# xmindflow/TransCeption

Measured on AMD Instinct MI355X. Metric: images/sec fwd+bwd at 224x224 B=16 per GPU, higher is better.
Workload: dtype bf16; 1 GPU; TransCeption (MSTransception) 224x224 B=16/GPU fwd+bwd+SGD, synthetic Synapse npz slices via the device loader, name-seeded random-init weights; global_batch=16, image_size=224, parallelism=dp1, headline_mode=loader, headline_degraded=False, launch_mode=hipGraph replay

## Files before the change

### include/transception_hip.h

```cpp
#ifndef TRANSCEPTION_HIP_H
#define TRANSCEPTION_HIP_H

#ifdef __cplusplus
extern "C" {
#endif

enum { TC_OK = 0, TC_ERR_ARG = -1, TC_ERR_LAUNCH = -2, TC_ERR_UNSUPPORTED = -3 };
enum { TC_F32 = 0, TC_BF16 = 1, TC_F16 = 2 };
enum { TC_ACT_NONE = 0, TC_ACT_HSWISH = 1, TC_ACT_COORD = 2, TC_ACT_SIGMOID = 3, TC_ACT_GELU = 4,
       TC_ACT_SCALE = 5 ,
       TC_ACT_RELU = 6   };

int tc_abi_version(void);

typedef struct TcGemm {
    const void* A; const void* B; void* C;
    const void* bias;
    const void* R;
    int M, N, K;
    int lda, ldb, ldc, ldr;
    int transA, transB;
    int nb1, nb2;
    long long sA1, sA2, sB1, sB2, sC1, sC2, sR1, sR2;
    float alpha;
    int accumulate;
    int act;
    int splitk;
    int dtype;
    int c_f32;
    int atomic;
    float* rowsum;
    long long sBias1, sRow1;
    int bgap_every;
    long long bgap;
    void* ws;
    long long ws_bytes;
    int ffn_mode, ffn_nchunk, ffn_chunk_n, ffn_ldd;
    float ffn_eps;
    const float* ffn_part; float* ffn_stat; const void* ffn_gamma; const void* ffn_beta; const void* ffn_d; float* ffn_part2;
    long long ffn_sRow1, ffn_sPar1;
    void* ffn_aout;
    float* bn_part; const float* bn_shift;
} TcGemm;
enum { TC_FFN_NONE = 0, TC_FFN_LN_A = 1, TC_FFN_LN_B = 2, TC_FFN_EP = 3 };
int tc_gemm(const TcGemm* g, void* stream);
int tc_gemm_pair(const TcGemm* a, const TcGemm* b, void* stream);
int tc_gemm_multi(const TcGemm* g, int n, void* stream);

int tc_colsum(const void* x, int rows, int cols, int ldx, int nb, long long sb, float* out, int accumulate, int dtype,
              void* stream);

int tc_layernorm_fwd(const void* x, int ldx, const void* gamma, const void* beta, void* y, int ldy,
                     float* mean, float* rstd, int rows, int C, float eps, int act, int groups, long long pstride,
                     int dtype, void* stream);
int tc_layernorm_bwd(const void* dy, int lddy, const void* x, int ldx, const void* gamma, const void* beta,
                     const float* mean, const float* rstd, void* dx, int lddx, const void* dres, int ldres,
                     float* dgamma, float* dbeta, int rows, int C, int act, int groups, long long pstride,
                     float* scratch, long long scratch_floats, int dtype, void* stream);
long long tc_layernorm_bwd_scratch_floats(int rows, int C, int groups);
typedef struct {
    const float* part;
    float* dgamma; float* dbeta;
    long long pstride;
    int nblk, C, groups;
} TcLnFold;
int tc_layernorm_bwd_nblk(int rows, int C);
int tc_layernorm_bwd_defer(const void* dy, int lddy, const void* x, int ldx, const void* gamma, const void* beta,
                           const float* mean, const float* rstd, void* dx, int lddx, const void* dres, int ldres,
                           float* dgamma, float* dbeta, int rows, int C, int act, int groups, long long pstride,
                           float* part, long long part_floats, int dtype, void* stream);
int tc_layernorm_fold(const TcLnFold* sites, int n, void* stream);
int tc_layernorm_bwd_params(const void* dy, int lddy, const void* x, int ldx, const void* gamma, const void* beta,
                            const float* mean, const float* rstd, float* dgamma, float* dbeta, int rows, int C, int act,
                            int groups, long long pstride, int dtype, void* stream);

int tc_layernorm_ps_fwd(const void* x, int ldx, const void* gamma, const void* beta, void* y, int ldy, float* mean, float* rstd,
                        int B, int H, int W, int p, int C, float eps, int dtype, void* stream);
int tc_layernorm_ps_bwd(const void* dy, int lddy, const void* x, int ldx, const void* gamma, const void* beta, const float* mean,
                        const float* rstd, void* dx, int lddx, float* dgamma, float* dbeta, int B, int H, int W, int p, int C,
                        float* scratch, long long scratch_floats, int dtype, void* stream);

int tc_ln_cls_supported(int C, int ncls, int dtype);
long long tc_ln_cls_scratch_floats(int rows, int ncls);
int tc_ln_cls_fwd(const void* x, int ldx, const void* gamma, const void* beta, const void* Wc, const void* bc, void* logits, int ldl,
                  float* mean, float* rstd, int B, int H, int W, int p, int C, int ncls, float eps, int dtype, void* stream);
int tc_ln_cls_bwd(const void* dl, int lddl, const void* x, int ldx, const void* gamma, const void* beta, const void* Wc, const float* mean,
                  const float* rstd, void* dx, int lddx, float* dgamma, float* dbeta, float* dWc, float* dbc, float* scratch,
                  long long scratch_floats, int B, int H, int W, int p, int C, int ncls, int dtype, void* stream);

int tc_dwconv_fwd(const void* x, int ldx, const void* w, const void* bias, void* y, int ldy,
                  int B, int H, int W, int C, int k, int stride, int add_input, int groups, long long wstride, int dtype,
                  void* stream);
int tc_dwconv_bwd_input(const void* dy, int lddy, const void* w, void* dx, int lddx,
                        int B, int H, int W, int C, int k, int stride, int add_input, int accumulate, int groups,
                        long long wstride, int dtype, void* stream);
int tc_dwconv_bwd_weight(const void* dy, int lddy, const void* x, int ldx, float* dw, float* db,
                         int B, int H, int W, int C, int k, int stride, int groups, long long wstride, void* ws,
                         long long ws_bytes, int dtype, void* stream);
typedef struct {
    const float* part; float* dw; float* db;
    float* dgamma; float* dbeta;
    long long wstride;
    int C, k, groups;
    int ch, chunks, gx, nt;
} TcDwFold;
long long tc_dwconv_bwd_plan(int B, int H, int W, int C, int k, int groups, int dtype, TcDwFold* site);
int tc_dw_fold(const TcDwFold* sites, int n, void* stream);
int tc_dwconv_bwd(const void* dy, int lddy, const void* x, int ldx, const void* w, void* dx, int lddx, float* dw, float* db, int B, int H,
                  int W, int C, int k, int add_input, int accumulate, int groups, long long wstride, void* ws, long long ws_bytes,
                  int dtype, void* stream);

typedef struct TcDwSeg {
    const void* x; const void* w; const void* bias; void* y; const void* dy; float* dw; float* db;
    int C; int k; int ldx; int ldy; int lddy; int B; int H; int W;
    float* stat;
} TcDwSeg;
int tc_dwconv_multi(const TcDwSeg* segs, int nseg, int mode, int add_input, int accumulate, int groups, long long wstride,
                    void* ws, long long ws_bytes, int dtype, void* stream);
long long tc_dwconv_multi_plan(const TcDwSeg* segs, int nseg, int groups, int dtype, TcDwFold* sites, long long* offs);

int tc_ffn_chunk(int C, int dtype);
int tc_ffn_dw_fwd(const void* x, int ldx, const void* w, const void* bias, void* y, int ldy, float* stat, int B, int H, int W,
                  int C, int groups, long long wstride, int dtype, void* stream);
typedef struct TcFfnSeg {
    const void* gp; const void* d; const void* h; void* dh; const float* stat; const float* part2; const void* w; const void* gamma;
    float* dw; float* db; float* dgamma; float* dbeta;
    int C, ldg, ldd, ldh, lddh, B, H, W, nch2;
} TcFfnSeg;
int tc_ffn_mid_bwd(const TcFfnSeg* segs, int nseg, int groups, long long wstride, void* ws, long long ws_bytes, int dtype,
                   void* stream);
// ... 263 lines not shown
```

### transception_amd/_lib.py

```python
from __future__ import annotations

import ctypes as C
import os

HERE = os.path.dirname(os.path.abspath(__file__))
LIB_PATH = os.environ.get("TC_LIB_PATH") or os.path.join(HERE, "libtransception_hip.so")

TC_F32, TC_BF16, TC_F16 = 0, 1, 2
ACT_NONE, ACT_HSWISH, ACT_COORD, ACT_SIGMOID, ACT_GELU, ACT_SCALE, ACT_RELU = 0, 1, 2, 3, 4, 5, 6
ABI_VERSION = 15
ATTN_DKV_SPLITS = 8

vp, i32, i64, f32, f64 = C.c_void_p, C.c_int, C.c_longlong, C.c_float, C.c_double


class TcGemm(C.Structure):
    _fields_ = [("A", vp), ("B", vp), ("C", vp), ("bias", vp), ("R", vp),
                ("M", i32), ("N", i32), ("K", i32),
                ("lda", i32), ("ldb", i32), ("ldc", i32), ("ldr", i32),
                ("transA", i32), ("transB", i32), ("nb1", i32), ("nb2", i32),
                ("sA1", i64), ("sA2", i64), ("sB1", i64), ("sB2", i64),
                ("sC1", i64), ("sC2", i64), ("sR1", i64), ("sR2", i64),
                ("alpha", f32), ("accumulate", i32), ("act", i32), ("splitk", i32), ("dtype", i32), ("c_f32", i32), ("atomic", i32), ("rowsum", vp), ("sBias1", i64), ("sRow1", i64),
                ("bgap_every", i32), ("bgap", i64), ("ws", vp), ("ws_bytes", i64),
                ("ffn_mode", i32), ("ffn_nchunk", i32), ("ffn_chunk_n", i32), ("ffn_ldd", i32), ("ffn_eps", f32),
                ("ffn_part", vp), ("ffn_stat", vp), ("ffn_gamma", vp), ("ffn_beta", vp), ("ffn_d", vp), ("ffn_part2", vp),
                ("ffn_sRow1", i64), ("ffn_sPar1", i64), ("ffn_aout", vp),
                ("bn_part", vp), ("bn_shift", vp)]


FFN_NONE, FFN_LN_A, FFN_LN_B, FFN_EP = 0, 1, 2, 3


class TcDwSeg(C.Structure):
    _fields_ = [("x", vp), ("w", vp), ("bias", vp), ("y", vp), ("dy", vp), ("dw", vp), ("db", vp), ("C", i32), ("k", i32),
                ("ldx", i32), ("ldy", i32), ("lddy", i32), ("B", i32), ("H", i32), ("W", i32), ("stat", vp)]


class TcDwFold(C.Structure):
    _fields_ = [("part", vp), ("dw", vp), ("db", vp), ("dgamma", vp), ("dbeta", vp), ("wstride", i64), ("C", i32), ("k", i32), ("groups", i32),
                ("ch", i32), ("chunks", i32), ("gx", i32), ("nt", i32)]


class TcLnFold(C.Structure):
    _fields_ = [("part", vp), ("dgamma", vp), ("dbeta", vp), ("pstride", i64), ("nblk", i32), ("C", i32), ("groups", i32)]


class TcFfnSeg(C.Structure):
    _fields_ = [("gp", vp), ("d", vp), ("h", vp), ("dh", vp), ("stat", vp), ("part2", vp), ("w", vp), ("gamma", vp),
                ("dw", vp), ("db", vp), ("dgamma", vp), ("dbeta", vp),
                ("C", i32), ("ldg", i32), ("ldd", i32), ("ldh", i32), ("lddh", i32), ("B", i32), ("H", i32), ("W", i32), ("nch2", i32)]


class TcFfnFused(C.Structure):
    _fields_ = [("x", vp), ("w1", vp), ("b1", vp), ("wd", vp), ("bd", vp), ("gamma", vp), ("beta", vp), ("w2", vp), ("b2", vp),
                ("res", vp), ("out", vp), ("h", vp), ("d", vp), ("a", vp), ("stat", vp),
                ("sres", i64), ("sout", i64), ("wstride", i64),
                ("ldx", i32), ("ldr", i32), ("ldo", i32), ("C", i32), ("B", i32), ("H", i32), ("W", i32), ("groups", i32), ("eps", f32),
                ("tile_h", i32), ("tile_w", i32), ("pre_gamma", vp), ("pre_beta", vp), ("pre_eps", f32)]


class TcFfnBwd(C.Structure):
    _fields_ = [("x", vp), ("dy", vp), ("d", vp), ("stat", vp),
                ("w1", vp), ("b1", vp), ("wd", vp), ("gamma", vp), ("beta", vp), ("w2", vp),
                ("dx", vp), ("gd", vp), ("part", vp), ("part_floats", i64),
                ("dw1", vp), ("db1", vp), ("dwd", vp), ("dbd", vp), ("dgamma", vp), ("dbeta", vp), ("dw2", vp), ("db2", vp),
                ("sdy", i64), ("wstride", i64),
                ("ldx", i32), ("lddy", i32), ("lddx", i32), ("C", i32), ("B", i32), ("H", i32), ("W", i32), ("groups", i32), ("acc_dx", i32),
                ("eps", f32), ("tile_h", i32), ("tile_w", i32),
                ("pre_gamma", vp), ("pre_beta", vp), ("dpre_gamma", vp), ("dpre_beta", vp), ("pre_eps", f32)]


class TcEffAtt(C.Structure):
    _fields_ = [("t", vp), ("gamma", vp), ("beta", vp),
                ("wk", vp), ("bk", vp), ("wq", vp), ("bq", vp), ("wv", vp), ("bv", vp), ("wr", vp), ("br", vp),
                ("out", vp), ("ctx", vp), ("kstat", vp), ("part", vp), ("part_floats", i64),
                ("dout", vp), ("dt", vp), ("g1", vp),
                ("dgamma", vp), ("dbeta", vp), ("dwk", vp), ("dbk", vp), ("dwq", vp), ("dbq", vp), ("dwv", vp), ("dbv", vp), ("dwr", vp), ("dbr", vp),
                ("ldt", i32), ("ldo", i32), ("lddo", i32), ("lddt", i32), ("acc_dt", i32), ("C", i32), ("B", i32), ("N", i32),
                ("eps", f32)]


class TcEwSeg(C.Structure):
    _fields_ = [("kind", i32), ("flag", i32), ("a", vp), ("b", vp), ("sa", i64), ("sb", i64),
                ("lda", i32), ("ldb", i32), ("n0", i32), ("n1", i32), ("n2", i32), ("n3", i32), ("n4", i32), ("reserved", i32)]


EW_PATCHIFY, EW_DEINTERLEAVE, EW_COPY = 0, 1, 2


class TcSliceAug(C.Structure):
    _fields_ = [("m", C.c_double * 6), ("disp", C.c_float * 32), ("alpha", f32), ("center", f32), ("noise_sigma", f32),
                ("noise_seed", C.c_uint), ("flags", i32), ("reserved", i32)]


TC_AUG_WARP, TC_AUG_LINEAR, TC_AUG_BLUR, TC_AUG_PIECEWISE = 1, 2, 4, 8
TC_AUG_SKIP, TC_AUG_FROM_RAW = 1 << 20, 1 << 21
TC_METRIC_NO_SOURCE = 1 << 28
TC_METRIC_SELECT_WORK_BYTES = 16448

SIGNATURES = {
    "tc_abi_version": [],
    "tc_gemm": [C.POINTER(TcGemm), vp],
    "tc_ew_multi": [C.POINTER(TcEwSeg), i32, i32, vp],
    "tc_gemm_pair": [C.POINTER(TcGemm), C.POINTER(TcGemm), vp],
    "tc_gemm_multi": [C.POINTER(TcGemm), i32, vp],
    "tc_colsum": [vp, i32, i32, i32, i32, i64, vp, i32, i32, vp],
    "tc_layernorm_fwd": [vp, i32, vp, vp, vp, i32, vp, vp, i32, i32, f32, i32, i32, i64, i32, vp],
    "tc_layernorm_bwd": [vp, i32, vp, i32, vp, vp, vp, vp, vp, i32, vp, i32, vp, vp, i32, i32, i32, i32, i64, vp, i64, i32, vp],
    "tc_layernorm_bwd_scratch_floats": [i32, i32, i32],
    "tc_layernorm_bwd_nblk": [i32, i32],
    "tc_dwconv_bwd_plan": [i32, i32, i32, i32, i32, i32, i32, vp],
    "tc_dwconv_multi_plan": [vp, i32, i32, i32, vp, vp],
    "tc_ffn_mid_plan": [vp, i32, i32, i32, vp, vp],
    "tc_dw_fold": [vp, i32, vp],
    "tc_layernorm_bwd_defer": [vp, i32, vp, i32, vp, vp, vp, vp, vp, i32, vp, i32, vp, vp, i32, i32, i32, i32, i64, vp, i64, i32, vp],
    "tc_layernorm_fold": [vp, i32, vp],
    "tc_layernorm_ps_fwd": [vp, i32, vp, vp, vp, i32, vp, vp, i32, i32, i32, i32, i32, f32, i32, vp],
    "tc_layernorm_ps_bwd": [vp, i32, vp, i32, vp, vp, vp, vp, vp, i32, vp, vp, i32, i32, i32, i32, i32, vp, i64, i32, vp],
    "tc_ln_cls_supported": [i32, i32, i32],
    "tc_ln_cls_scratch_floats": [i32, i32],
    "tc_ln_cls_fwd": [vp, i32, vp, vp, vp, vp, vp, i32, vp, vp, i32, i32, i32, i32, i32, i32, f32, i32, vp],
    "tc_ln_cls_bwd": [vp, i32, vp, i32, vp, vp, vp, vp, vp, vp, i32, vp, vp, vp, vp, vp, i64, i32, i32, i32, i32, i32, i32, i32, vp],
    "tc_layernorm_bwd_params": [vp, i32, vp, i32, vp, vp, vp, vp, vp, vp, i32, i32, i32, i32, i64, i32, vp],
    "tc_dwconv_fwd": [vp, i32, vp, vp, vp, i32, i32, i32, i32, i32, i32, i32, i32, i32, i64, i32, vp],
    "tc_dwconv_bwd_input": [vp, i32, vp, vp, i32, i32, i32, i32, i32, i32, i32, i32, i32, i32, i64, i32, vp],
    "tc_dwconv_bwd_weight": [vp, i32, vp, i32, vp, vp, i32, i32, i32, i32, i32, i32, i32, i64, vp, i64, i32, vp],
    "tc_dwconv_bwd": [vp, i32, vp, i32, vp, vp, i32, vp, vp, i32, i32, i32, i32, i32, i32, i32, i32, i64, vp, i64, i32, vp],
    "tc_dwconv_multi": [C.POINTER(TcDwSeg), i32, i32, i32, i32, i32, i64, vp, i64, i32, vp],
    "tc_ffn_chunk": [i32, i32],
    "tc_ffn_dw_fwd": [vp, i32, vp, vp, vp, i32, vp, i32, i32, i32, i32, i32, i64, i32, vp],
    "tc_ffn_mid_bwd": [C.POINTER(TcFfnSeg), i32, i32, i64, vp, i64, i32, vp],
    "tc_ffn_fused_supported": [i32, i32],
    "tc_ffn_fused_fwd": [C.POINTER(TcFfnFused), i32, vp],
    "tc_ffn_fused_bwd_supported": [i32, i32],
    "tc_ffn_fused_bwd_scratch_floats": [i32, i32],
    "tc_ffn_fused_bwd": [C.POINTER(TcFfnBwd), i32, vp],
    "tc_effatt_supported": [i32, i32],
    "tc_effatt_scratch_floats": [i32, i32, i32],
    "tc_effatt_fwd": [C.POINTER(TcEffAtt), i32, vp],
    "tc_effatt_bwd": [C.POINTER(TcEffAtt), i32, vp],
    "tc_bn_scratch_floats": [i32, i32],
    "tc_bn_fwd": [vp, i32, vp, vp, vp, vp, vp, i32, vp, i32, vp, vp, vp, i32, i32, f32, f32, i32, i32, i32, i32, vp],
    "tc_bn_bwd": [vp, i32, vp, i32, vp, vp, vp, vp, vp, i32, vp, vp, vp, i32, i32, i32, i32, i32, vp],
    "tc_softmax_scratch_floats": [i32, i32, i32],
    "tc_softmax_fwd": [vp, vp, vp, i32, i64, i64, i32, i32, i32, i32, i32, i32, vp],
    "tc_softmax_bwd": [vp, vp, vp, vp, i32, i64, i64, i64, i32, i32, i32, i32, i32, i32, i32, i32, vp],
    "tc_attn_fwd": [vp, i32, i64, vp, i32, vp, i32, i64, vp, i32, i64, vp, i32, i32, i32, f32, i32, vp],
    "tc_attn_bwd": [vp, i32, i64, vp, i32, vp, i32, i64, vp, i32, i64, vp, i32, i64, vp, vp, vp, i32, i64, vp, i32,
                    vp, i32, i64, i32, i32, i32, i32, f32, i32, vp],
    "tc_attn_fwd_seg": [vp, i32, vp, i32, vp, i32, i64, vp, i32, vp, i32, i32, C.POINTER(i32), i32, f32, i32, i32, vp],
    "tc_attn_bwd_seg": [vp, i32, vp, i32, vp, i32, i64, vp, i32, vp, i32, vp, vp, vp, vp, i32, vp, i32, vp, i32, i64, i32, i32,
                        C.POINTER(i32), i32, f32, i32, i32, vp],
    "tc_fma3_fwd": [vp, i32, vp, i32, vp, i32, vp, i32, i32, i32, f32, i32, vp],
    "tc_fma3_bwd": [vp, i32, vp, i32, vp, i32, vp, i32, vp, i32, i32, vp, i32, i32, i32, f32, i32, vp],
    "tc_add": [vp, i32, vp, i32, vp, i32, i32, i32, i32, vp],
    "tc_sigmoid_bwd": [vp, vp, vp, i64, i32, vp],
    "tc_copy3d": [vp, i64, i32, vp, i64, i32, i32, i32, i32, i32, i32, vp],
    "tc_transpose": [vp, vp, i32, i32, i32, i32, vp],
    "tc_chan_pool_fwd": [vp, i32, vp, i32, i32, i32, i32, vp],
    "tc_chan_pool_bwd": [vp, vp, i32, i32, i32, i32, i32, i32, vp],
    "tc_chan_gate_fwd": [vp, i32, vp, vp, i32, i32, i32, i32, i32, vp],
    "tc_chan_gate_bwd": [vp, i32, vp, i32, vp, vp, i32, i32, vp, i32, i32, i32, i32, vp],
    "tc_relu_fwd": [vp, vp, i64, i32, vp],
    "tc_relu_bwd": [vp, vp, vp, i64, i32, vp],
    "tc_chan_pool2_fwd": [vp, i32, vp, vp, i32, i32, i32, i32, vp],
    "tc_chan_pool2_bwd": [vp, vp, vp, i32, i32, i32, i32, i32, i32, vp],
    "tc_pix_stats_fwd": [vp, i32, vp, vp, i32, i32, i32, vp],
    "tc_pix_stats_bwd": [vp, vp, vp, i32, i32, i32, i32, i32, vp],
    "tc_sa_conv_fwd": [vp, vp, vp, vp, i32, i32, i32, i32, i32, vp],
    "tc_sa_conv_bwd": [vp, vp, vp, vp, vp, vp, vp, i32, i32, i32, i32, i32, vp],
    "tc_pix_gate_fwd": [vp, i32, vp, vp, i32, i32, i32, i32, vp],
    "tc_pix_gate_bwd": [vp, i32, vp, i32, vp, vp, i32, i32, vp, i32, i32, i32, vp],
    "tc_cam_att_fwd": [vp, i32, vp, i32, i32, i32, i32, vp],
    "tc_cam_apply_fwd": [vp, i32, vp, vp, vp, i32, i32, i32, i32, i32, vp],
    "tc_cam_bwd": [vp, i32, vp, i32, vp, vp, vp, vp, vp, i32, i32, i32, i32, i32, i32, vp],
    "tc_gamma_res_fwd": [vp, i32, vp, i32, vp, vp, i32, i32, i32, i32, vp],
    "tc_gamma_res_bwd": [vp, i32, vp, i32, vp, vp, i32, vp, i32, i32, vp, i32, i32, i32, vp],
    "tc_gelu_fwd": [vp, vp, i64, i32, vp],
    "tc_gelu_bwd": [vp, vp, vp, i64, i32, vp],
    "tc_coord_pool_fwd": [vp, vp, i32, i32, i32, i32, i32, vp],
    "tc_coord_pool_bwd": [vp, vp, i32, i32, i32, i32, i32, i32, vp],
    "tc_coord_gate_fwd": [vp, vp, vp, i32, i32, i32, i32, i32, vp],
    "tc_coord_gate_bwd": [vp, vp, vp, vp, i32, vp, i32, i32, i32, i32, i32, vp],
    "tc_pixel_shuffle": [vp, vp, i32, i32, i32, i32, i32, i32, i32, vp],
    "tc_patchify": [vp, i64, i32, vp, i32, i32, i32, i32, i32, i32, i32, vp],
    "tc_sr_deinterleave": [vp, vp, i64, i32, i32, i32, i32, i32, i32, i32, vp],
    "tc_stem_im2col": [vp, vp, i32, i32, i32, i32, i32, i32, vp],
    "tc_window_rows": [vp, i32, vp, i32, i32, i32, i32, i32, i32, i32, i32, i32, i32, i32, vp],
    "tc_dropout": [vp, vp, i64, f32, vp, C.c_uint, i32, vp],
    "tc_im2col3s2": [vp, i32, i32, i32, vp, i32, i32, i32, i32, i32, i32, vp],
    "tc_col2im3s2": [vp, i32, vp, i32, i32, i32, i32, i32, i32, i32, vp],
    "tc_seg_loss_fwd": [vp, vp, vp, vp, i32, i32, i32, i32, vp],
    "tc_factor_att_stats_floats": [i32, i32, i32],
    "tc_factor_att_fwd": [vp, vp, vp, i32, vp, i32, vp, i32, vp, i32, i32, i32, i32, f32, i32, vp],
    "tc_factor_att_bwd": [vp, vp, vp, i32, vp, i32, vp, i32, vp, vp, vp, vp, i32, i32, i32, i32, vp, i32, i32, i32, i32, i32, f32, i32, vp],
    "tc_argmax_counts": [vp, vp, vp, vp, i32, i32, i32, i32, vp],
    "tc_metric_hist_bins": [i32, i32, i32],
    "tc_metric_surfaces": [vp, vp, vp, vp, vp, i32, i32, i32, i32, i32, vp],
    "tc_metric_edt": [vp, i32, vp, i32, i32, i32, i32, vp],
    "tc_metric_hist": [vp, vp, vp, vp, i32, vp, i64, i32, i32, i32, i32, vp],
    "tc_metric_select": [vp, i64, i32, vp, vp],
    "tc_metric_edt_f64": [vp, i32, vp, i32, i32, i32, i32, f64, f64, f64, vp],
    "tc_metric_select_f64": [vp, vp, vp, vp, i32, i32, i32, i32, i32, vp, vp, vp],
    "tc_seg_loss_bwd": [vp, vp, vp, vp, i32, i32, i32, f32, f32, f32, f32, vp, i32, vp],
    "tc_seg_loss_fwd_tok": [vp, i32, vp, vp, vp, i32, i32, i32, i32, vp],
    "tc_seg_loss_bwd_tok": [vp, vp, i32, vp, vp, vp, i32, i32, i32, i32, f32, f32, f32, f32, vp, i32, vp],
    "tc_seg_loss_value": [vp, i32, C.c_double, C.c_double, C.c_double, vp, vp],
    "tc_seg_loss_fwd_w": [vp, i32, vp, vp, i32, vp, vp, i32, i32, i32, i32, vp],
    "tc_seg_loss_value_w": [vp, vp, i32, C.c_double, C.c_double, vp, vp],
    "tc_seg_loss_bwd_w": [vp, vp, i32, vp, vp, i32, vp, vp, i32, i32, i32, i32, f32, f32, f32, vp, i32, vp],
    "tc_slice_augment": [vp, vp, vp, vp, vp, i32, i32, i32, vp],
    "tc_slice_augment_chain": [vp, vp, vp, i32, i32, vp, vp, vp, vp, i32, i32, i32, vp],
    "tc_spline_prefilter": [vp, vp, i32, i32, i32, vp],
    "tc_zoom_normalize": [vp, vp, vp, vp, vp, i32, i32, i32, i32, i32, f32, f32, vp],
    "tc_sgd_step": [vp, vp, vp, i64, f32, vp, f32, f32, f32, i32, vp],
    "tc_sgd_step_multi": [vp, vp, vp, vp, i32, i64, f32, vp, f32, f32, f32, i32, vp, f32, vp, i32, vp],
    "tc_sgd_step_multi_scaled": [vp, vp, vp, vp, i32, i64, f32, vp, f32, f32, f32, i32, vp, f32, vp, i32, vp, vp],
    "tc_loss_scale_update": [vp, vp, f32, f32, i32, f32, f32, vp],
    "tc_grad_sumsq": [vp, i64, vp, vp],
    "tc_fill_f32": [vp, i64, f32, vp],
    "tc_cast": [vp, vp, i64, i32, i32, vp],
    "tc_seg_marker": [i32, vp],
    "tc_im2col_dil": [vp, i32, vp, i32, i32, i32, i32, i32, i32, i32, i32, i32, i32, vp],
    "tc_col2im_dil": [vp, i32, vp, i32, i32, i32, i32, i32, i32, i32, i32, i32, i32, i32, vp],
    "tc_nearest_concat_fwd": [vp, i64, vp, i64, i32, vp, i32, i32, i32, i32, i32, i32, i32, i32, vp],
    "tc_nearest_concat_bwd": [vp, i32, vp, i64, vp, i64, i32, i32, i32, i32, i32, i32, i32, i32, i32, vp],
    "tc_linear_ln_supported": [i32, i32],
    "tc_linear_ln_fwd": [vp, i32, vp, vp, i64, vp, i32, vp, vp, i64, vp, i32, vp, i32, vp, vp, i32, i32, i32, f32, i32, vp],
    "tc_ripm_supported": [i32, i32],
    "tc_ripm_tiles": [i32, i32, i32],
    "tc_ripm_fwd": [vp, i32, i32, vp, i32, vp, vp, vp, vp, vp, vp, f32, f32, i32, vp, i32, vp, vp, vp, i32, vp, i32, vp, vp, i32, i32, i32, i32, i32, i32, vp],
    "tc_mhca_att_supported": [i32, i32, i32],
    "tc_dw_ln_supported": [i32, i32],
    "tc_dw_ln_fwd": [vp, i32, vp, vp, i64, vp, vp, i64, vp, i32, vp, i32, vp, vp, i32, i32, i32, i32, i32, f32, i32, vp],
    "tc_mhca_att_bwd_supported": [i32, i32, i32],
    "tc_mhca_att_bwd": [vp, i32, vp, i32, vp, i32, vp, vp, i32, i32, i32, i32, vp, vp, vp, vp, vp, vp, vp, vp, vp, i64, i32, i32, i32, i32, i32, f32, i32, vp],
    "tc_mhca_att_fwd": [vp, i32, vp, vp, vp, vp, vp, vp, vp, vp, i64, vp, i32, vp, i32, vp, i32, vp, i32, i32, i32, i32, i32, f32, i32, vp],
}
_RET = {"tc_ln_cls_scratch_floats": i64, "tc_ffn_fused_bwd_scratch_floats": i64, "tc_effatt_scratch_floats": i64, "tc_bn_scratch_floats": i64, "tc_softmax_scratch_floats": i64, "tc_layernorm_bwd_scratch_floats": i64, "tc_dwconv_bwd_plan": i64, "tc_dwconv_multi_plan": i64, "tc_ffn_mid_plan": i64, "tc_factor_att_stats_floats": i64, "tc_metric_hist_bins": i64}
_RAW = {"tc_abi_version", "tc_ln_cls_supported", "tc_ln_cls_scratch_floats", "tc_linear_ln_supported", "tc_ripm_supported", "tc_ripm_tiles", "tc_mhca_att_supported", "tc_dw_ln_supported", "tc_mhca_att_bwd_supported", "tc_effatt_supported", "tc_effatt_scratch_floats", "tc_ffn_chunk", "tc_ffn_fused_supported", "tc_ffn_fused_bwd_supported", "tc_ffn_fused_bwd_scratch_floats", "tc_bn_scratch_floats", "tc_softmax_scratch_floats", "tc_layernorm_bwd_scratch_floats", "tc_layernorm_bwd_nblk", "tc_dwconv_bwd_plan", "tc_dwconv_multi_plan", "tc_ffn_mid_plan", "tc_factor_att_stats_floats", "tc_metric_hist_bins"}


class TcError(RuntimeError):
    pass


class _Lib:
    calls = 0

    def __init__(self, path: str = LIB_PATH):
        if not os.path.exists(path):
            raise TcError(f"{path} is missing: build it with `python -m transception_amd.build` "
                          "(there is no CPU/PyTorch fallback for the TransCeption hot path)")
        self.path = path
        self.cdll = C.CDLL(path)
        for name, args in SIGNATURES.items():
            fn = getattr(self.cdll, name)
            fn.argtypes = args
            fn.restype = _RET.get(name, i32)
            setattr(self, name, fn if name in _RAW else self._checked(name, fn))
        v = self.cdll.tc_abi_version()
        if v != ABI_VERSION:
            raise TcError(f"ABI mismatch: library {v}, host {ABI_VERSION}")

    @staticmethod
    def _checked(name, fn):
        def call(*a):
            _Lib.calls += 1
            rc = fn(*a)
            if rc != 0:
                raise TcError(f"{name} failed with status {rc}")
        call.__name__ = name
        return call


_lib = None


def lib() -> _Lib:
    global _lib
    if _lib is None:
        _lib = _Lib()
    return _lib
```

### transception_amd/csrc/gemm.hip

```cpp
#include "tc_common.h"
#include <algorithm>
#include <type_traits>
#include <cstdlib>

typedef float f32x16 __attribute__((ext_vector_type(16)));
typedef __bf16 bf16x8 __attribute__((ext_vector_type(8)));
typedef _Float16 f16x8 __attribute__((ext_vector_type(8)));

template <typename H> struct HalfOps;
template <> struct HalfOps<bf16_t> {
    typedef bf16x8 v8;
    static __device__ __forceinline__ f32x16 mfma(v8 a, v8 b, f32x16 c) { return __builtin_amdgcn_mfma_f32_32x32x16_bf16(a, b, c, 0, 0, 0); }
};
template <> struct HalfOps<f16_t> {
    typedef f16x8 v8;
    static __device__ __forceinline__ f32x16 mfma(v8 a, v8 b, f32x16 c) { return __builtin_amdgcn_mfma_f32_32x32x16_f16(a, b, c, 0, 0, 0); }
};

namespace {

static inline unsigned fdiv_make(long long d, unsigned long long nmax) {
    return (d > 1 && nmax * (unsigned long long)d < (1ull << 32)) ? (unsigned)((1ull << 32) / (unsigned long long)d + 1) : 0u;
}
__device__ __forceinline__ int fdiv(int n, int d, unsigned m) { return d == 1 ? n : (m ? (int)__umulhi((unsigned)n, m) : n / d); }

struct GemmDev {
    const void* A; const void* B; void* C; const void* bias; const void* R;
    int M, N, K, lda, ldb, ldc, ldr;
    int nb2, splitk, kchunk;
    unsigned m_splitk, m_nb2, m_gx;
    long long sA1, sA2, sB1, sB2, sC1, sC2, sR1, sR2;
    float alpha; int accumulate, act;
    unsigned char vecA, vecB, vecC, atomic;
    short vec8C;
    short xcd;
    float* rowsum;
    long long sBias1, sRow1;
    float* ws_part; int* ws_cnt; short fix_group, fix_ngroups;
    int bgap_every; long long bgap;
    struct {
        int mode, nchunk, chunk_n, ldd, sRow1, sPar1;
        float eps;
        const float* part; float* stat; const void* gamma; const void* beta; const void* d; float* part2;
    } ffn;
    __device__ __host__ float* bn_part() const { return ffn.mode == 4 ? ffn.part2 : nullptr; }
    __device__ __host__ const float* bn_shift() const { return ffn.part; }
};
constexpr int GEMM_BN_STATS = 4;

template <typename H> __device__ __forceinline__ void bf8_unpack(const uint4& r, float* o) {
    unpack2<H>(r.x, o[0], o[1]); unpack2<H>(r.y, o[2], o[3]); unpack2<H>(r.z, o[4], o[5]); unpack2<H>(r.w, o[6], o[7]);
}
template <typename H> __device__ __forceinline__ uint4 bf8_pack(const float* o) {
    return make_uint4(pack2<H>(o[0], o[1]), pack2<H>(o[2], o[3]), pack2<H>(o[4], o[5]), pack2<H>(o[6], o[7]));
}
template <typename H> __device__ __forceinline__ uint4 ffn_ln_gelu8(const uint4& v, float mean, float rstd, const float* g, const float* b) {
    float x[8];
    bf8_unpack<H>(v, x);
#pragma unroll
    for (int e = 0; e < 8; e += 2) {
        const tc_f32x2 xv = {x[e], x[e + 1]}, gv = {g[e], g[e + 1]}, bv = {b[e], b[e + 1]};
        const tc_f32x2 u = gelu_poly2((xv - mean) * rstd * gv + bv);
        x[e] = u.x; x[e + 1] = u.y;
    }
    return bf8_pack<H>(x);
}
__device__ __forceinline__ float4 ffn_ln_gelu4(const float4& v, float mean, float rstd, const float4& g, const float4& b) {
    return make_float4(gelu_f((v.x - mean) * rstd * g.x + b.x), gelu_f((v.y - mean) * rstd * g.y + b.y),
                       gelu_f((v.z - mean) * rstd * g.z + b.z), gelu_f((v.w - mean) * rstd * g.w + b.w));
}
template <int BM>
__device__ __forceinline__ void ffn_finalize_stats(const GemmDev& p, int b1, int m0, bool write_out, float2* s_stat) {
    constexpr int LPR = 256 / BM;
    const int tid = threadIdx.x, r = tid / LPR, q = tid % LPR, row = m0 + r;
    const long long rbase = (long long)b1 * p.ffn.sRow1;
    const int nch = p.ffn.nchunk;
    const float cn = (float)p.ffn.chunk_n, inv_cn = 1.0f / cn, invC = 1.0f / (cn * (float)nch);
    const float2* pp = reinterpret_cast<const float2*>(p.ffn.part) + (rbase + (row < p.M ? row : 0)) * nch;
    float sm = 0.f, m2 = 0.f;
    constexpr int PMAX = 16;
    if (nch <= PMAX * LPR) {
        float2 t[PMAX];
#pragma unroll
        for (int e = 0; e < PMAX; ++e) t[e] = pp[min(q + e * LPR, nch - 1)];
#pragma unroll
        for (int e = 0; e < PMAX; ++e) if (q + e * LPR < nch) sm += t[e].x;
        sm = tc_group_sum<LPR>(sm);
        const float mean_ = sm * invC;
#pragma unroll
        for (int e = 0; e < PMAX; ++e) if (q + e * LPR < nch) { const float dm = t[e].x * inv_cn - mean_; m2 += t[e].y + cn * dm * dm; }
    } else {
        for (int k = q; k < nch; k += LPR) sm += pp[k].x;
        sm = tc_group_sum<LPR>(sm);
        const float mean_ = sm * invC;
        for (int k = q; k < nch; k += LPR) { const float2 t = pp[k]; const float dm = t.x * inv_cn - mean_; m2 += t.y + cn * dm * dm; }
    }
    const float mean = sm * invC;
    m2 = tc_group_sum<LPR>(m2);
    const float rstd = rsqrtf(m2 * invC + p.ffn.eps);
    if (q == 0) {
        s_stat[r] = make_float2(mean, rstd);
        if (write_out && row < p.M) reinterpret_cast<float2*>(p.ffn.stat)[rbase + row] = make_float2(mean, rstd);
    }
    __syncthreads();
}
template <typename T> __device__ __forceinline__ float ffn_ep1(float v, float d, float mean, float rstd, float g, float b, float& s1, float& s2) {
    const float xh = (d - mean) * rstd;
    const float gp = v * gelu_grad_fT<T>(xh * g + b);
    s1 += gp * g; s2 += gp * g * xh;
    return gp;
}

template <int TM, int TN>
__device__ __forceinline__ bool splitk_fixup(const GemmDev& p, f32x16 (&acc)[TM][TN], int tile, int ks, int& grp) {
    const int G = p.fix_group, tid = threadIdx.x;
    grp = ks / G;
    const int g0 = grp * G, gm = min(G, p.splitk - g0);
    if (gm == 1) return true;
    constexpr int NV = TM * TN * 16;
    float* part = p.ws_part + ((long long)tile * p.splitk + ks) * (NV * 256) + tid;
#pragma unroll
    for (int i = 0; i < TM; ++i)
#pragma unroll
        for (int j = 0; j < TN; ++j)
#pragma unroll
            for (int r = 0; r < 16; ++r)
                __hip_atomic_store(part + ((i * TN + j) * 16 + r) * 256, acc[i][j][r], __ATOMIC_RELAXED, __HIP_MEMORY_SCOPE_AGENT);
    __builtin_amdgcn_s_waitcnt(0);
    __builtin_amdgcn_fence(__ATOMIC_RELEASE, "workgroup");
    __syncthreads();
    __shared__ int s_last;
// ... 217 lines not shown
                    const int lr = part * 16 + r;
                    const float v = (m0 + lr < p.M) ? ldf<H>(stage + lr * LDS_ + cc) - sh : 0.f;
                    s1 += v; s2 += v * v;
                }
            }
            red[part * 64 + cc] = s1; red[256 + part * 64 + cc] = s2;
            __syncthreads();
            if (threadIdx.x < 64 && col < p.N) {
                const int T = (p.M + BM - 1) / BM, t = m0 / BM;
                bnp[p.N + (long long)t * p.N + col] = red[cc] + red[64 + cc] + red[128 + cc] + red[192 + cc];
                bnp[p.N + (long long)(T + t) * p.N + col] = red[256 + cc] + red[320 + cc] + red[384 + cc] + red[448 + cc];
                if (t == 0) bnp[col] = sh;
            }
        }
    }
}

template <typename H, int BM, int BN, int TM, int TN>
__device__ __forceinline__ void epilogue_rows_lds_ep(const GemmDev& p, f32x16 (&acc)[TM][TN], int b1, int m0, int n0, int wr, int wc, int lane,
                                                     bf16_t* stage_raw, const uint4 rd0, const uint4 rd1, int bx, int gx) {
    constexpr int LDS_ = BN + 8, WM = BM / 2, WN = BN / 2, CPR = BN / 8;
    H* stage = reinterpret_cast<H*>(stage_raw);
    H* dt = stage + BM * LDS_;
    float2* srow = reinterpret_cast<float2*>(dt + BM * LDS_);
    const long long rbase = (long long)b1 * p.ffn.sRow1;
    const H* gam = reinterpret_cast<const H*>(p.ffn.gamma) + (long long)b1 * p.ffn.sPar1;
    const H* bet = reinterpret_cast<const H*>(p.ffn.beta) + (long long)b1 * p.ffn.sPar1;
    const float2* stat = reinterpret_cast<const float2*>(p.ffn.stat) + rbase;
    const int h = lane >> 5;
    __syncthreads();
    {
        const int lr = threadIdx.x / CPR, lc = (threadIdx.x % CPR) * 8;
        *reinterpret_cast<uint4*>(dt + lr * LDS_ + lc) = rd0;
        *reinterpret_cast<uint4*>(dt + (lr + 256 / CPR) * LDS_ + lc) = rd1;
    }
    __syncthreads();
#pragma unroll
    for (int i = 0; i < TM; ++i) {
        const int lr = wr * WM + i * 32 + (lane & 31), row = m0 + lr;
        const float2 st = stat[row < p.M ? row : 0];
        float s1 = 0.f, s2 = 0.f;
#pragma unroll
        for (int j = 0; j < TN; ++j)
#pragma unroll
            for (int g = 0; g < 4; ++g) {
                const int lc = wc * WN + j * 32 + 8 * g + 4 * h, col = n0 + lc;
                float v[4];
#pragma unroll
                for (int e = 0; e < 4; ++e) v[e] = p.alpha * acc[i][j][4 * g + e];
                if (row < p.M && col < p.N) {
                    const float4 d4 = ld4<H>(dt + lr * LDS_ + lc), g4 = ld4<H>(gam + col), b4 = ld4<H>(bet + col);
                    {
                        const tc_f32x2 va = {v[0], v[1]}, vb = {v[2], v[3]};
                        const tc_f32x2 ga = {g4.x, g4.y}, gb = {g4.z, g4.w};
                        const tc_f32x2 xa = (tc_f32x2{d4.x, d4.y} - st.x) * st.y, xb = (tc_f32x2{d4.z, d4.w} - st.x) * st.y;
                        const tc_f32x2 pa = va * gelu_grad_f2_fast(xa * ga + tc_f32x2{b4.x, b4.y});
                        const tc_f32x2 pb = vb * gelu_grad_f2_fast(xb * gb + tc_f32x2{b4.z, b4.w});
                        const tc_f32x2 qa = pa * ga, qb = pb * gb, ra = qa * xa, rb = qb * xb;
                        s1 += (qa.x + qa.y) + (qb.x + qb.y);
                        s2 += (ra.x + ra.y) + (rb.x + rb.y);
                        v[0] = pa.x; v[1] = pa.y; v[2] = pb.x; v[3] = pb.y;
                    }
                }
                st4<H>(stage + lr * LDS_ + lc, make_float4(v[0], v[1], v[2], v[3]));
            }
        s1 += __shfl_xor(s1, 32, 64); s2 += __shfl_xor(s2, 32, 64);
        if (h == 0) srow[wc * BM + lr] = make_float2(s1, s2);
    }
    __syncthreads();
    H* C = reinterpret_cast<H*>(p.C) + b1 * p.sC1;
#pragma unroll
    for (int it = 0; it < BM * CPR / 256; ++it) {
        const int idx = threadIdx.x + it * 256, lr = idx / CPR, lc = (idx - lr * CPR) * 8;
        const int row = m0 + lr, col = n0 + lc;
        if (row < p.M && col < p.N)
            *reinterpret_cast<uint4*>(C + (long long)row * p.ldc + col) = *reinterpret_cast<const uint4*>(stage + lr * LDS_ + lc);
    }
    if (threadIdx.x < BM && m0 + threadIdx.x < p.M) {
        const float2 a = srow[threadIdx.x], b = srow[BM + threadIdx.x];
        reinterpret_cast<float2*>(p.ffn.part2)[(rbase + m0 + threadIdx.x) * gx + bx] = make_float2(a.x + b.x, a.y + b.y);
    }
}

__device__ __forceinline__ float4 load_strip(const float* base, int ld, int x, int k, int X, int K, bool trans, bool vec) {
    float4 v = make_float4(0.f, 0.f, 0.f, 0.f);
    if (!trans) {
        if (x < X) {
            const float* p = base + (long long)x * ld + k;
            if (vec && k + 3 < K) v = *reinterpret_cast<const float4*>(p);
            else {
                if (k + 0 < K) v.x = p[0];
                if (k + 1 < K) v.y = p[1];
                if (k + 2 < K) v.z = p[2];
                if (k + 3 < K) v.w = p[3];
            }
        }
    } else {
        if (k < K) {
            const float* p = base + (long long)k * ld + x;
            if (vec && x + 3 < X) v = *reinterpret_cast<const float4*>(p);
            else {
                if (x + 0 < X) v.x = p[0];
                if (x + 1 < X) v.y = p[1];
                if (x + 2 < X) v.z = p[2];
                if (x + 3 < X) v.w = p[3];
            }
        }
    }
    return v;
}

template <typename TC, int BM, int BN, bool TA, bool TB, int FFN = 0>
__global__ __launch_bounds__(256) void gemm_kernel(GemmDev p) {
    constexpr int BK = 16, LDT = BK + 1;
    constexpr int WM = BM / 2, WN = BN / 2, TM = WM / 32, TN = WN / 32;
    constexpr int SA = BM * BK / 4 / 256, SB = BN * BK / 4 / 256;
    static_assert(SA >= 1 && SB >= 1, "tile too small");
    static_assert(FFN == 0 || (BM == 64 && BN == 64), "the MixFFN hooks run on 64x64 tiles");
    static_assert(FFN != TC_FFN_LN_A || !TA, "LN_A transforms rows of a row-major A");
    static_assert(FFN != TC_FFN_LN_B || !TB, "LN_B transforms rows of a [K,N] B");
    __shared__ float As[BM * LDT];
    __shared__ float Bs[BN * LDT];
    __shared__ float2 s_ffn[FFN ? 2 * 64 : 1];

    const int tid = threadIdx.x, lane = tid & 63, wave = tid >> 6;
    const int wr = wave >> 1, wc = wave & 1;
    int z = blockIdx.z;
    const int ks = z % p.splitk; z /= p.splitk;
    const int b2 = z % p.nb2, b1 = z / p.nb2;
    const int m0 = blockIdx.y * BM, n0 = blockIdx.x * BN;
    const int kbeg = ks * p.kchunk;
    const int kend = min(p.K, kbeg + p.kchunk);

    const float* A = reinterpret_cast<const float*>(p.A) + b1 * p.sA1 + b2 * p.sA2;
    const float* B = reinterpret_cast<const float*>(p.B) + b1 * p.sB1 + b2 * p.sB2;
    const float* gam = FFN ? reinterpret_cast<const float*>(p.ffn.gamma) + (long long)b1 * p.ffn.sPar1 : nullptr;
    const float* bet = FFN ? reinterpret_cast<const float*>(p.ffn.beta) + (long long)b1 * p.ffn.sPar1 : nullptr;
    const float2* fstat = FFN ? reinterpret_cast<const float2*>(p.ffn.stat) + (long long)b1 * p.ffn.sRow1 : nullptr;

    f32x16 acc[TM][TN];
#pragma unroll
    for (int i = 0; i < TM; ++i)
#pragma unroll
        for (int j = 0; j < TN; ++j)
#pragma unroll
            for (int r = 0; r < 16; ++r) acc[i][j][r] = 0.f;

    float a_mean = 0.f, a_rstd = 0.f;
    float4 hg = make_float4(0.f, 0.f, 0.f, 0.f), hb = hg;
    float2 hst = make_float2(0.f, 0.f);
    if constexpr (FFN == TC_FFN_LN_A) {
        ffn_finalize_stats<BM>(p, b1, m0, blockIdx.x == 0 && ks == 0, s_ffn);
        const float2 st = s_ffn[tid / (BK / 4)];
        a_mean = st.x; a_rstd = st.y;
    }
    if constexpr (FFN == TC_FFN_LN_B) {
        const int col = n0 + (tid % (BN / 4)) * 4;
        if (col + 3 < p.N) { hg = *reinterpret_cast<const float4*>(gam + col); hb = *reinterpret_cast<const float4*>(bet + col); }
    }

    float4 ra[SA], rb[SB];
    auto fetch = [&](int k0) __attribute__((always_inline)) {
#pragma unroll
        for (int i = 0; i < SA; ++i) {
            const int f = tid + i * 256;
            if (!TA) { const int row = f / (BK / 4), kq = f % (BK / 4);
// ... 60 lines not shown
        if (k0 + BK < kend) fetch(k0 + BK);
        if (do_rowsum) {
#pragma unroll
            for (int kk = 0; kk < BK; ++kk) rsum += As[tid * LDT + kk];
        }
        const float* ap = &As[(wr * WM + (lane & 31)) * LDT + (lane >> 5)];
        const float* bp = &Bs[(wc * WN + (lane & 31)) * LDT + (lane >> 5)];
#pragma unroll
        for (int kk = 0; kk < BK; kk += 2) {
            float a[TM], b[TN];
#pragma unroll
            for (int i = 0; i < TM; ++i) a[i] = ap[i * 32 * LDT + kk];
#pragma unroll
            for (int j = 0; j < TN; ++j) b[j] = bp[j * 32 * LDT + kk];
#pragma unroll
            for (int i = 0; i < TM; ++i)
#pragma unroll
                for (int j = 0; j < TN; ++j)
                    acc[i][j] = __builtin_amdgcn_mfma_f32_32x32x2f32(a[i], b[j], acc[i][j], 0, 0, 0);
        }
        __syncthreads();
    }
    if (do_rowsum && m0 + tid < p.M) atomicAdd(p.rowsum + b1 * p.sRow1 + m0 + tid, rsum);
    bool first = (ks == 0), atomic = p.atomic;
    if (p.fix_group) {
        int grp;
        if (!splitk_fixup<TM, TN>(p, acc, (int)(((blockIdx.z / p.splitk) * gridDim.y + blockIdx.y) * gridDim.x + blockIdx.x), ks, grp)) return;
        first = (grp == 0); atomic = p.fix_ngroups > 1;
    }
    if constexpr (FFN == TC_FFN_EP)
        epilogue_cols<float, TC, TM, TN, true>(p, acc, b1, b2, first, atomic, m0 + wr * WM, n0 + wc * WN, lane, s_ffn, wr * WM, wc, m0,
                                               (int)blockIdx.x, (int)gridDim.x);
    else
        epilogue_cols<float, TC, TM, TN>(p, acc, b1, b2, first, atomic, m0 + wr * WM, n0 + wc * WN, lane);
}

__device__ __forceinline__ bool strip_whole(int x, int k, int X, int K, bool trans) {
    return trans ? (k < K && x + 7 < X) : (x < X && k + 7 < K);
}
__device__ __forceinline__ uint4 strip_raw(const bf16_t* base, const bf16_t* safe, int ld, int x, int k, int X, int K, bool trans) {
    const long long off = trans ? (long long)k * ld + x : (long long)x * ld + k;
    return *reinterpret_cast<const uint4*>(strip_whole(x, k, X, K, trans) ? base + off : safe);
}
__device__ __forceinline__ uint4 strip_tail(const bf16_t* base, int ld, int x, int k, int X, int K, bool trans) {
    union { uint4 v; bf16_t e[8]; } u;
    u.v = make_uint4(0u, 0u, 0u, 0u);
    const bf16_t* p = base + (trans ? (long long)k * ld + x : (long long)x * ld + k);
#pragma unroll
    for (int i = 0; i < 8; ++i) if (trans ? (x + i < X) : (k + i < K)) u.e[i] = p[i];
    return u.v;
}
__device__ __forceinline__ uint4 load_strip8(const bf16_t* base, int ld, int x, int k, int X, int K, bool trans, bool vec) {
    const bool in = trans ? (k < K) : (x < X);
    if (!in) return make_uint4(0u, 0u, 0u, 0u);
    if (vec && strip_whole(x, k, X, K, trans))
        return *reinterpret_cast<const uint4*>(base + (trans ? (long long)k * ld + x : (long long)x * ld + k));
    return strip_tail(base, ld, x, k, X, K, trans);
}

__device__ __forceinline__ int gemm_krow(int k) { return (k & ~15) | ((k & 3) << 2) | ((k >> 2) & 3); }
typedef short s16x4_t __attribute__((ext_vector_type(4)));
typedef short s16x8_t __attribute__((ext_vector_type(8)));
template <typename V8> __device__ __forceinline__ V8 ld_frag_tr(const bf16_t* lo, const bf16_t* hi) {
    const s16x4_t a = __builtin_amdgcn_ds_read_tr16_b64_v4i16((s16x4_t __attribute__((address_space(3)))*)(lo));
    const s16x4_t b = __builtin_amdgcn_ds_read_tr16_b64_v4i16((s16x4_t __attribute__((address_space(3)))*)(hi));
    return __builtin_bit_cast(V8, (s16x8_t)__builtin_shufflevector(a, b, 0, 1, 2, 3, 4, 5, 6, 7));
}

#ifdef TC_GEMM_TIMING
__device__ unsigned long long g_gemm_dbg[1024 * 8];
__device__ unsigned int g_gemm_dbg_n;
#define GSTAMP(k) do { if (gs_ >= 0) { const long long t_ = __builtin_readcyclecounter(); g_gemm_dbg[gs_ * 8 + 1 + (k)] = (unsigned long long)(t_ - gt_); gt_ = t_; } } while (0)
#define GSTAMP_INIT() int gs_ = -1; long long gt_ = 0; \
    if (threadIdx.x == 0 && (blockIdx.x + 7 * blockIdx.y + 13 * blockIdx.z) % 61 == 0) { gs_ = (int)(atomicAdd(&g_gemm_dbg_n, 1u) & 1023u); \
        g_gemm_dbg[gs_ * 8] = (TA ? 4 : 0) + (TB ? 2 : 0) + (sizeof(TC) == 4 ? 1 : 0) + 8 * FFN + 1000ull * (unsigned long long)((kend_for_stamp)); gt_ = __builtin_readcyclecounter(); }
#else
#define GSTAMP(k)
#define GSTAMP_INIT()
#endif
template <typename H, typename TC, int BM, int BN, bool TA, bool TB, bool DB, int FFN = 0>
__device__ __forceinline__ void gemm_bf16_body(const GemmDev& p, const int bx, const int by, const int bz, const int gx, const int gy,
                                               bf16_t (*As)[BM * (64 + 8)], bf16_t (*Bs)[BN * (64 + 8)]) {
    constexpr int BK = 64, LDT = BK + 8;
    static_assert(FFN == 0 || (BM == 64 && BN == 64 && DB), "the MixFFN hooks run on 64x64 tiles with the double-buffered LDS");
    static_assert(FFN != TC_FFN_LN_A || !TA, "LN_A transforms rows of a row-major A");
    static_assert(FFN != TC_FFN_LN_B || !TB, "LN_B transforms rows of a [K,N] B");
    static_assert(FFN != TC_FFN_EP || sizeof(TC) == 2, "EP writes a bf16 C");
    constexpr bool SWAP = sizeof(TC) == 2;
    constexpr int WM = BM / 2, WN = BN / 2, TM = WM / 32, TN = WN / 32;
    constexpr int SA = BM * BK / 8 / 256, SB = BN * BK / 8 / 256;
    static_assert(SA >= 1 && SB >= 1, "tile too small");

    const int tid = threadIdx.x, lane = tid & 63, wave = tid >> 6;
    const int wr = wave >> 1, wc = wave & 1;
    int z = bz;
    const int zq = fdiv(z, p.splitk, p.m_splitk);
    const int ks = z - zq * p.splitk; z = zq;
    const int b1 = fdiv(z, p.nb2, p.m_nb2), b2 = z - b1 * p.nb2;
    const int m0 = by * BM, n0 = bx * BN;
    const int kbeg = ks * p.kchunk;
    const int kend = min(p.K, kbeg + p.kchunk);
    const int kend_for_stamp = kend - kbeg; (void)kend_for_stamp;
    GSTAMP_INIT();

    const bf16_t* A = reinterpret_cast<const bf16_t*>(p.A) + b1 * p.sA1 + b2 * p.sA2;
    const bf16_t* B = reinterpret_cast<const bf16_t*>(p.B) + b1 * p.sB1 + b2 * p.sB2;

    f32x16 acc[TM][TN];
#pragma unroll
    for (int i = 0; i < TM; ++i)
#pragma unroll
        for (int j = 0; j < TN; ++j)
#pragma unroll
            for (int r = 0; r < 16; ++r) acc[i][j][r] = 0.f;

    auto a_xy = [&](int i, int k0, int& x, int& k) __attribute__((always_inline)) {
        const int f = tid + i * 256;
        if (!TA) { x = m0 + f / (BK / 8); k = k0 + (f % (BK / 8)) * 8; }
        else { k = k0 + f / (BM / 8); x = m0 + (f % (BM / 8)) * 8; }
    };
    auto b_xy = [&](int i, int k0, int& x, int& k) __attribute__((always_inline)) {
        const int f = tid + i * 256;
        if (TB) { x = n0 + f / (BK / 8); k = k0 + (f % (BK / 8)) * 8; }
        else { k = k0 + f / (BN / 8); x = n0 + (f % (BN / 8)) * 8; }
    };
    auto b_base = [&](int k0) __attribute__((always_inline)) { return (!TB && p.bgap_every) ? B + (long long)(k0 / p.bgap_every) * p.bgap : B; };
    const bf16_t* gam = FFN ? reinterpret_cast<const bf16_t*>(p.ffn.gamma) + (long long)b1 * p.ffn.sPar1 : nullptr;
    const bf16_t* bet = FFN ? reinterpret_cast<const bf16_t*>(p.ffn.beta) + (long long)b1 * p.ffn.sPar1 : nullptr;
    const float2* fstat = FFN ? reinterpret_cast<const float2*>(p.ffn.stat) + (long long)b1 * p.ffn.sRow1 : nullptr;
    __shared__ float2 s_ffn[FFN == TC_FFN_LN_A ? BM : 1];
    float a_mean[SA], a_rstd[SA], fg[8], fb[8];
    bf16_t* aout = (FFN == TC_FFN_LN_A && p.ffn.d && bx == 0) ? reinterpret_cast<bf16_t*>(const_cast<void*>(p.ffn.d)) + (long long)b1 * p.ffn.sRow1 * p.ffn.ldd
                                                               : nullptr;
    uint4 rd0 = make_uint4(0u, 0u, 0u, 0u), rd1 = rd0;
    if constexpr (FFN == TC_FFN_LN_A) {
        ffn_finalize_stats<BM>(p, b1, m0, bx == 0 && ks == 0, s_ffn);
#pragma unroll
        for (int i = 0; i < SA; ++i) { const float2 st = s_ffn[(tid + i * 256) / (BK / 8)]; a_mean[i] = st.x; a_rstd[i] = st.y; }
    }
    if constexpr (FFN == TC_FFN_LN_B) {
        const int col = n0 + (tid % (BN / 8)) * 8;
        const int cc = col + 7 < p.N ? col : 0;
        bf8_unpack<H>(*reinterpret_cast<const uint4*>(gam + cc), fg);
        bf8_unpack<H>(*reinterpret_cast<const uint4*>(bet + cc), fb);
    }
    if constexpr (FFN == TC_FFN_EP) {
        const bf16_t* dmap = reinterpret_cast<const bf16_t*>(p.ffn.d) + (long long)b1 * p.ffn.sRow1 * p.ffn.ldd;
        static_assert(BM * BN / 8 / 256 == 2 || FFN != TC_FFN_EP, "two pieces per thread");
        const int lr = tid / (BN / 8), lc = (tid % (BN / 8)) * 8;
        const bool in0 = m0 + lr < p.M && n0 + lc < p.N, in1 = m0 + lr + 256 / (BN / 8) < p.M && n0 + lc < p.N;
        rd0 = *reinterpret_cast<const uint4*>(in0 ? dmap + (long long)(m0 + lr) * p.ffn.ldd + n0 + lc : dmap);
        rd1 = *reinterpret_cast<const uint4*>(in1 ? dmap + (long long)(m0 + lr + 256 / (BN / 8)) * p.ffn.ldd + n0 + lc : dmap);
    }
    auto fetch = [&](auto FT, uint4 (&ra)[SA], uint4 (&rb)[SB], uint4 (&rh)[2], int k0) __attribute__((always_inline)) {
        constexpr bool FAST = decltype(FT)::value;
        int x, k;
#pragma unroll
        for (int i = 0; i < SA; ++i) {
            a_xy(i, k0, x, k);
            if constexpr (FAST) ra[i] = strip_raw(A, A, p.lda, x, k, p.M, kend, TA);
            else ra[i] = load_strip8(A, p.lda, x, k, p.M, kend, TA, p.vecA);
        }
        const bf16_t* Bk = b_base(k0);
#pragma unroll
        for (int i = 0; i < SB; ++i) {
            b_xy(i, k0, x, k);
            if constexpr (FAST) rb[i] = strip_raw(Bk, B, p.ldb, x, k, p.N, kend, !TB);
// ... 44 lines not shown
            else if constexpr (FFN == TC_FFN_LN_B) { if (!strip_whole(x, k, p.N, kend, !TB)) v = make_uint4(0u, 0u, 0u, 0u); }
            if (TB) { const int row = f / (BK / 8), kq = f % (BK / 8); *reinterpret_cast<uint4*>(&bs[row * LDT + kq * 8]) = v; }
            else { const int kl = f / (BN / 8), nq = f % (BN / 8); *reinterpret_cast<uint4*>(&bs[gemm_krow(kl) * PB + nq * 8]) = v; }
        }
    };
    float rsum = 0.f;
    const bool do_rowsum = p.rowsum && bx == 0 && tid < BM;
    auto compute = [&](const bf16_t* as, const bf16_t* bs) __attribute__((always_inline)) {
        if (do_rowsum) {
#pragma unroll
            for (int kk = 0; kk < BK; ++kk) rsum += ldf<H>(reinterpret_cast<const H*>(TA ? as + kk * PA + tid : as + tid * LDT + kk));
        }
        const int h = lane >> 5, gi = lane & 15, gq = (lane >> 4) & 1;
        const bf16_t* ap = TA ? &as[(2 * h + 4 * (gi >> 2)) * PA + wr * WM + 16 * gq + 4 * (gi & 3)] : &as[(wr * WM + (lane & 31)) * LDT + 8 * h];
        const bf16_t* bp = !TB ? &bs[(2 * h + 4 * (gi >> 2)) * PB + wc * WN + 16 * gq + 4 * (gi & 3)] : &bs[(wc * WN + (lane & 31)) * LDT + 8 * h];
#pragma unroll
        for (int kk = 0; kk < BK; kk += 16) {
            typedef typename HalfOps<H>::v8 V8;
            V8 a[TM], b[TN];
#pragma unroll
            for (int i = 0; i < TM; ++i) {
                if constexpr (TA) a[i] = ld_frag_tr<V8>(ap + kk * PA + i * 32, ap + (kk + 1) * PA + i * 32);
                else a[i] = *reinterpret_cast<const V8*>(ap + i * 32 * LDT + kk);
            }
#pragma unroll
            for (int j = 0; j < TN; ++j) {
                if constexpr (!TB) b[j] = ld_frag_tr<V8>(bp + kk * PB + j * 32, bp + (kk + 1) * PB + j * 32);
                else b[j] = *reinterpret_cast<const V8*>(bp + j * 32 * LDT + kk);
            }
#pragma unroll
            for (int i = 0; i < TM; ++i)
#pragma unroll
                for (int j = 0; j < TN; ++j)
                    acc[i][j] = SWAP ? HalfOps<H>::mfma(b[j], a[i], acc[i][j])
                                     : HalfOps<H>::mfma(a[i], b[j], acc[i][j]);
        }
    };

    auto kloop = [&](auto FT) __attribute__((always_inline)) {
    constexpr bool FAST = decltype(FT)::value;
    uint4 ra0[SA], rb0[SB], ra1[SA], rb1[SB], rh0[2], rh1[2];
    if (!DB) {
        if (kbeg < kend) fetch(FT, ra0, rb0, rh0, kbeg);
        for (int k0 = kbeg; k0 < kend; k0 += BK) {
            stage(FT, ra0, rb0, rh0, k0, As[0], Bs[0]);
            __syncthreads();
            if (k0 + BK < kend) fetch(FT, ra0, rb0, rh0, k0 + BK);
            compute(As[0], Bs[0]);
            __syncthreads();
        }
    } else if (kbeg < kend) {
        fetch(FT, ra0, rb0, rh0, kbeg);
        if (FAST || kbeg + BK < kend) fetch(FT, ra1, rb1, rh1, kbeg + BK);
        stage(FT, ra0, rb0, rh0, kbeg, As[0], Bs[0]);
        __syncthreads();
        if (FAST || kbeg + 2 * BK < kend) fetch(FT, ra0, rb0, rh0, kbeg + 2 * BK);
        for (int k0 = kbeg;; k0 += 2 * BK) {
            const bool has1 = k0 + BK < kend;
            if (has1) stage(FT, ra1, rb1, rh1, k0 + BK, As[DB ? 1 : 0], Bs[DB ? 1 : 0]);
            compute(As[0], Bs[0]);
            if (!has1) break;
            __syncthreads();
            if (FAST || k0 + 3 * BK < kend) fetch(FT, ra1, rb1, rh1, k0 + 3 * BK);
            const bool has2 = k0 + 2 * BK < kend;
            if (has2) stage(FT, ra0, rb0, rh0, k0 + 2 * BK, As[0], Bs[0]);
            compute(As[DB ? 1 : 0], Bs[DB ? 1 : 0]);
            if (!has2) break;
            __syncthreads();
            if (FAST || k0 + 4 * BK < kend) fetch(FT, ra0, rb0, rh0, k0 + 4 * BK);
        }
    }
    };
    const bool fast = p.vecA && p.vecB && ((kend - kbeg) % 8 == 0 || (TA && !TB)) && (!TA || p.M % 8 == 0) && (TB || p.N % 8 == 0);
    GSTAMP(0);
    if (fast) kloop(std::true_type{}); else kloop(std::false_type{});
    GSTAMP(1);
    if (do_rowsum && m0 + tid < p.M) atomicAdd(p.rowsum + b1 * p.sRow1 + m0 + tid, rsum);
    bool first = (ks == 0), atomic = p.atomic;
    if (p.fix_group) {
        int grp;
        if (!splitk_fixup<TM, TN>(p, acc, (zq * gy + by) * gx + bx, ks, grp)) return;
        first = (grp == 0); atomic = p.fix_ngroups > 1;
    }
    if constexpr (FFN == TC_FFN_EP) {
        static_assert(FFN != TC_FFN_EP || 2 * BM * (BN + 8) + 2 * BM * 4 <= 2 * (BM + BN) * (64 + 8), "C stage + d tile + row sums must fit");
        epilogue_rows_lds_ep<H, BM, BN, TM, TN>(p, acc, b1, m0, n0, wr, wc, lane, &As[0][0], rd0, rd1, bx, gx);
    } else if constexpr (SWAP) {
        if (p.vec8C && !p.accumulate && !atomic && first) {
            static_assert((BM * (BN + 8)) <= (DB ? 2 : 1) * (BM + BN) * (64 + 8), "staging tile must fit the operand buffers");
            epilogue_rows_lds<H, BM, BN, TM, TN>(p, acc, b1, b2, m0, n0, wr, wc, lane, &As[0][0]);
        } else {
            epilogue_rows<H, TC, TM, TN>(p, acc, b1, b2, first, atomic, m0 + wr * WM, n0 + wc * WN, lane);
        }
    } else {
        epilogue_cols<H, TC, TM, TN>(p, acc, b1, b2, first, atomic, m0 + wr * WM, n0 + wc * WN, lane);
    }
    GSTAMP(2);
}

__device__ __forceinline__ void tc_xcd_tile(int& bx, int& by, const int gx, const int gy, const unsigned mgx) {
    const int T = gx * gy, L = bx + gx * by;
    const int xcd = L & 7, slot = L >> 3, q = T >> 3, r = T & 7;
    const int t = xcd * q + min(xcd, r) + slot;
    by = fdiv(t, gx, mgx);
    bx = t - by * gx;
}

#ifndef GEMM_OCC64
#define GEMM_OCC64 5
#endif
template <typename H, typename TC, int BM, int BN, bool TA, bool TB, bool DB, int FFN = 0>
__global__ __launch_bounds__(256, (BM == 64 && BN == 64) ? GEMM_OCC64 : 2) void gemm_bf16_kernel(GemmDev p) {
    __shared__ __attribute__((aligned(16))) bf16_t smem[(DB ? 2 : 1) * (BM + BN) * (64 + 8)];
    int tbx = blockIdx.x, tby = blockIdx.y;
    if (p.xcd & 1) tc_xcd_tile(tbx, tby, gridDim.x, gridDim.y, p.m_gx);
    gemm_bf16_body<H, TC, BM, BN, TA, TB, DB, FFN>(p, tbx, tby, blockIdx.z, gridDim.x, gridDim.y,
                                                reinterpret_cast<bf16_t(*)[BM * (64 + 8)]>(smem),
                                                reinterpret_cast<bf16_t(*)[BN * (64 + 8)]>(smem + (DB ? 2 : 1) * BM * (64 + 8)));
}

struct GemmPairDev { GemmDev a, b; int nA, gxA, gyA, gxB, gyB; unsigned mgxA, mgyA, mgxB, mgyB; };
template <typename H>
__global__ __launch_bounds__(256, 2) void gemm_pair_kernel(GemmPairDev q) {
    __shared__ __attribute__((aligned(16))) bf16_t smem[2 * (64 + 64) * (64 + 8)];
    bf16_t(*As)[64 * (64 + 8)] = reinterpret_cast<bf16_t(*)[64 * (64 + 8)]>(smem);
    bf16_t(*Bs)[64 * (64 + 8)] = reinterpret_cast<bf16_t(*)[64 * (64 + 8)]>(smem + 2 * 64 * (64 + 8));
    const int nB = (int)gridDim.x - q.nA;
    int lin = (int)blockIdx.x < nB ? (int)blockIdx.x + q.nA : (int)blockIdx.x - nB;
    if (lin < q.nA) {
        const int l1 = fdiv(lin, q.gxA, q.mgxA);
        int bx = lin - l1 * q.gxA;
        const int bz = fdiv(l1, q.gyA, q.mgyA);
        int by = l1 - bz * q.gyA;
        if (q.a.xcd & 1) tc_xcd_tile(bx, by, q.gxA, q.gyA, q.mgxA);
        if (q.a.ffn.mode == TC_FFN_EP) gemm_bf16_body<H, H, 64, 64, false, false, true, TC_FFN_EP>(q.a, bx, by, bz, q.gxA, q.gyA, As, Bs);
        else gemm_bf16_body<H, H, 64, 64, false, false, true>(q.a, bx, by, bz, q.gxA, q.gyA, As, Bs);
    } else {
        lin -= q.nA;
        if (q.b.xcd & 2) {
            const int xcd = lin & 7, slot = lin >> 3, qq = nB >> 3, r = nB & 7;
            lin = xcd * qq + min(xcd, r) + slot;
        }
        const int l1 = fdiv(lin, q.gxB, q.mgxB), bx = lin - l1 * q.gxB, bz = fdiv(l1, q.gyB, q.mgyB), by = l1 - bz * q.gyB;
        if (q.b.ffn.mode == TC_FFN_LN_B) gemm_bf16_body<H, float, 64, 64, true, false, true, TC_FFN_LN_B>(q.b, bx, by, bz, q.gxB, q.gyB, As, Bs);
        else gemm_bf16_body<H, float, 64, 64, true, false, true>(q.b, bx, by, bz, q.gxB, q.gyB, As, Bs);
    }
}

constexpr int GEMM_MULTI_MAX = 12;
static_assert(sizeof(GemmDev) * GEMM_MULTI_MAX + 20 * GEMM_MULTI_MAX + 8 <= 4096, "kernel argument block");
struct GemmMultiDev { GemmDev p[GEMM_MULTI_MAX]; int blk0[GEMM_MULTI_MAX], gx[GEMM_MULTI_MAX], gy[GEMM_MULTI_MAX], kind[GEMM_MULTI_MAX]; unsigned mgy[GEMM_MULTI_MAX]; int n; };
template <typename H>
__global__ __launch_bounds__(256, 4) void gemm_multi_kernel(GemmMultiDev q) {
    __shared__ __attribute__((aligned(16))) bf16_t smem[2 * (64 + 64) * (64 + 8)];
    bf16_t(*As)[64 * (64 + 8)] = reinterpret_cast<bf16_t(*)[64 * (64 + 8)]>(smem);
    bf16_t(*Bs)[64 * (64 + 8)] = reinterpret_cast<bf16_t(*)[64 * (64 + 8)]>(smem + 2 * 64 * (64 + 8));
    int lin = blockIdx.x, i = 0;
    for (int j = 1; j < q.n; ++j) if (lin >= q.blk0[j]) i = j;
    lin -= q.blk0[i];
    if (q.p[i].xcd & 2) {
        const int ni = (i + 1 < q.n ? q.blk0[i + 1] : (int)gridDim.x) - q.blk0[i];
        const int xcd = lin & 7, slot = lin >> 3, qq = ni >> 3, r = ni & 7;
        lin = xcd * qq + min(xcd, r) + slot;
    }
    const int gx = q.gx[i], gy = q.gy[i];
    const unsigned mgx = q.p[i].m_gx;
    const int l1 = fdiv(lin, gx, mgx), bz = fdiv(l1, gy, q.mgy[i]);
    int bx = lin - l1 * gx, by = l1 - bz * gy;
    if ((q.p[i].xcd & 1) && q.kind[i] != 2 && q.kind[i] != 5) tc_xcd_tile(bx, by, gx, gy, mgx);
    const GemmDev p = q.p[i];
    if (q.kind[i] == 0) gemm_bf16_body<H, H, 64, 64, false, true, true>(p, bx, by, bz, gx, gy, As, Bs);
    else if (q.kind[i] == 1) gemm_bf16_body<H, H, 64, 64, false, false, true>(p, bx, by, bz, gx, gy, As, Bs);
    else if (q.kind[i] == 2) gemm_bf16_body<H, float, 64, 64, true, false, true>(p, bx, by, bz, gx, gy, As, Bs);
    else if (q.kind[i] == 3) gemm_bf16_body<H, H, 64, 64, false, true, true, TC_FFN_LN_A>(p, bx, by, bz, gx, gy, As, Bs);
    else if (q.kind[i] == 4) gemm_bf16_body<H, H, 64, 64, false, false, true, TC_FFN_EP>(p, bx, by, bz, gx, gy, As, Bs);
    else gemm_bf16_body<H, float, 64, 64, true, false, true, TC_FFN_LN_B>(p, bx, by, bz, gx, gy, As, Bs);
}

template <typename T, typename TC, int BM, int BN, bool TA, bool TB>
void launch_one(const GemmDev& d, dim3 grid, hipStream_t s) {
    if constexpr (sizeof(T) == 4) hipLaunchKernelGGL((gemm_kernel<TC, BM, BN, TA, TB>), grid, dim3(256), 0, s, d);
    else if (d.kchunk > 128) hipLaunchKernelGGL((gemm_bf16_kernel<T, TC, BM, BN, TA, TB, true>), grid, dim3(256), 0, s, d);
    else hipLaunchKernelGGL((gemm_bf16_kernel<T, TC, BM, BN, TA, TB, false>), grid, dim3(256), 0, s, d);
}

template <typename T>
int launch_ffn(const GemmDev& d, dim3 grid, hipStream_t s) {
    if constexpr (sizeof(T) == 4) {
        if (d.ffn.mode == TC_FFN_LN_A) hipLaunchKernelGGL((gemm_kernel<float, 64, 64, false, true, TC_FFN_LN_A>), grid, dim3(256), 0, s, d);
        else if (d.ffn.mode == TC_FFN_LN_B) hipLaunchKernelGGL((gemm_kernel<float, 64, 64, true, false, TC_FFN_LN_B>), grid, dim3(256), 0, s, d);
        else hipLaunchKernelGGL((gemm_kernel<float, 64, 64, false, false, TC_FFN_EP>), grid, dim3(256), 0, s, d);
    } else {
        if (d.ffn.mode == TC_FFN_LN_A) hipLaunchKernelGGL((gemm_bf16_kernel<T, T, 64, 64, false, true, true, TC_FFN_LN_A>), grid, dim3(256), 0, s, d);
        else if (d.ffn.mode == TC_FFN_LN_B) hipLaunchKernelGGL((gemm_bf16_kernel<T, float, 64, 64, true, false, true, TC_FFN_LN_B>), grid, dim3(256), 0, s, d);
        else hipLaunchKernelGGL((gemm_bf16_kernel<T, T, 64, 64, false, false, true, TC_FFN_EP>), grid, dim3(256), 0, s, d);
    }
    return tc_launch_status();
}

template <typename T, typename TC, int BM, int BN>
int launch(const GemmDev& d, int transA, int transB, dim3 grid, hipStream_t s) {
    if (!transA && transB) launch_one<T, TC, BM, BN, false, true>(d, grid, s);
    else if (!transA && !transB) launch_one<T, TC, BM, BN, false, false>(d, grid, s);
    else if (transA && !transB) launch_one<T, TC, BM, BN, true, false>(d, grid, s);
    else launch_one<T, TC, BM, BN, true, true>(d, grid, s);
    return tc_launch_status();
}

template <typename T>
bool gemm_plan(const TcGemm* g, GemmDev& d, dim3& grid, bool& use128_out, bool force64 = false) {
    d.A = g->A; d.B = g->B; d.C = g->C; d.bias = g->bias; d.R = g->R;
    d.M = g->M; d.N = g->N; d.K = g->K; d.lda = g->lda; d.ldb = g->ldb; d.ldc = g->ldc; d.ldr = g->ldr;
    d.nb2 = g->nb2; d.splitk = g->splitk;
    d.sA1 = g->sA1; d.sA2 = g->sA2; d.sB1 = g->sB1; d.sB2 = g->sB2;
    d.sC1 = g->sC1; d.sC2 = g->sC2; d.sR1 = g->sR1; d.sR2 = g->sR2;
    d.alpha = g->alpha; d.accumulate = g->accumulate; d.act = g->act;
    d.rowsum = g->rowsum;
    d.sBias1 = g->sBias1; d.sRow1 = g->sRow1;
    d.bgap_every = g->bgap_every; d.bgap = g->bgap;
    d.ffn.mode = g->ffn_mode; d.ffn.nchunk = g->ffn_nchunk; d.ffn.chunk_n = g->ffn_chunk_n; d.ffn.ldd = g->ffn_ldd;
    d.ffn.sRow1 = (int)g->ffn_sRow1; d.ffn.sPar1 = (int)g->ffn_sPar1; d.ffn.eps = g->ffn_eps;
    d.ffn.part = g->ffn_part; d.ffn.stat = g->ffn_stat; d.ffn.gamma = g->ffn_gamma; d.ffn.beta = g->ffn_beta;
    d.ffn.d = g->ffn_mode == TC_FFN_LN_A ? g->ffn_aout : g->ffn_d;
    d.ffn.part2 = g->ffn_part2;
    if (g->bn_part && !g->ffn_mode) { d.ffn.mode = GEMM_BN_STATS; d.ffn.part2 = g->bn_part; d.ffn.part = g->bn_shift; }
    if (g->ffn_mode || g->bn_part) force64 = true;
    constexpr int VEC = 16 / (int)sizeof(T);
    auto aligned = [&](const void* ptr, int ld, long long s1, long long s2) {
        return ((uintptr_t)ptr % 16 == 0) && (ld % VEC == 0) && (s1 % VEC == 0) && (s2 % VEC == 0);
    };
    d.vecA = aligned(g->A, g->lda, g->sA1, g->sA2);
    d.vecB = aligned(g->B, g->ldb, g->sB1, g->sB2);
    {
        const int csz = g->c_f32 ? 4 : (int)sizeof(T);
        const bool cok = ((uintptr_t)g->C % (4 * csz) == 0) && (g->ldc % 4 == 0) && (g->sC1 % 4 == 0) && (g->sC2 % 4 == 0);
        const bool rok = !g->R || (((uintptr_t)g->R % (4 * sizeof(T)) == 0) && (g->ldr % 4 == 0) && (g->sR1 % 4 == 0) && (g->sR2 % 4 == 0));
        d.vecC = cok && rok;
        d.vec8C = !g->c_f32 && sizeof(T) == 2 && cok && rok && ((uintptr_t)g->C % 16 == 0) && (g->ldc % 8 == 0) && (g->sC1 % 8 == 0) &&
                  (g->sC2 % 8 == 0) && (g->N % 8 == 0);
    }
    const int nb = g->nb1 * g->nb2;
    const long long big = (long long)((g->M + 127) / 128) * ((g->N + 127) / 128) * nb;
    constexpr long long thr128 = 100000;
    const bool use128 = !force64 && big >= thr128 && g->M >= 96 && g->N >= 96;
    const int BM = use128 ? 128 : 64, BN = use128 ? 128 : 64;
    constexpr int BK = sizeof(T) == 4 ? 16 : 64;
    constexpr int CNT_BYTES = 16384, PART_BYTES = 64 * 64 * 4, FIX_GROUP = 16;
    const long long tiles64 = (long long)((g->M + 63) / 64) * ((g->N + 63) / 64) * nb;
    const long long slots = (g->ws && g->ws_bytes > CNT_BYTES && (uintptr_t)g->ws % 16 == 0) ? (g->ws_bytes - CNT_BYTES) / PART_BYTES : 0;
    int want = g->splitk;
    bool fix = false;
    if (!use128 && slots > 0) {
#ifndef GEMM_AS_TILES
#define GEMM_AS_TILES 384
#define GEMM_AS_TARGET 512
#define GEMM_AS_KPER 256
#endif
        if (want == 1 && !g->atomic && g->ffn_mode != TC_FFN_EP && !g->bn_part && g->K >= 2 * GEMM_AS_KPER && tiles64 <= GEMM_AS_TILES) {
            long long sk = GEMM_AS_TARGET / tiles64;
            if (sk > g->K / GEMM_AS_KPER) sk = g->K / GEMM_AS_KPER;
            if (sk > FIX_GROUP) sk = FIX_GROUP;
            if (sk >= 2 && tiles64 * sk <= slots) { want = (int)sk; fix = true; }
        } else if (want > 128) {
            fix = tiles64 * want <= slots && tiles64 * ((want + FIX_GROUP - 1) / FIX_GROUP) <= CNT_BYTES / 4;
        }
    }
    int kchunk = (g->K + want - 1) / want;
    kchunk = (kchunk + BK - 1) / BK * BK;
    d.kchunk = kchunk;
    d.splitk = (g->K + kchunk - 1) / kchunk;
    if (d.splitk < 1) d.splitk = 1;
    d.fix_group = 0; d.fix_ngroups = 1; d.ws_part = nullptr; d.ws_cnt = nullptr;
    if (fix && d.splitk > 1) {
        d.fix_group = FIX_GROUP;
        d.fix_ngroups = (d.splitk + FIX_GROUP - 1) / FIX_GROUP;
        d.ws_cnt = reinterpret_cast<int*>(g->ws);
        d.ws_part = reinterpret_cast<float*>(reinterpret_cast<char*>(g->ws) + CNT_BYTES);
    }
    d.atomic = ((d.splitk > 1 && !d.fix_group) || g->atomic) ? 1 : 0;
    grid = dim3((g->N + BN - 1) / BN, (g->M + BM - 1) / BM, nb * d.splitk);
    d.m_splitk = fdiv_make(d.splitk, 65536); d.m_nb2 = fdiv_make(d.nb2, 65536);
    d.m_gx = fdiv_make(grid.x, (unsigned long long)grid.x * grid.y * grid.z);
    d.xcd = (grid.x > 1 && (long long)grid.x * grid.y >= 64) ? 1 : 0;
    use128_out = use128;
    if (g->bn_part) {
        if (sizeof(T) != 2 || g->c_f32 || g->accumulate || g->atomic || d.splitk != 1 || nb != 1 || !d.vec8C || g->ffn_mode || g->act != TC_ACT_NONE)
            return false;
    }
    if (g->ffn_mode) {
        if (!d.vecA || !d.vecB || (g->ffn_mode != TC_FFN_LN_B && g->K % VEC) || g->N % VEC || g->nb2 != 1 || (uintptr_t)g->ffn_gamma % 16 || (uintptr_t)g->ffn_beta % 16 ||
            g->ffn_sPar1 % VEC)
            return false;
        if (g->ffn_mode == TC_FFN_LN_A && (g->transA || !g->transB || g->c_f32 || g->K != g->ffn_nchunk * g->ffn_chunk_n ||
                                           (g->ffn_aout && ((uintptr_t)g->ffn_aout % 16 || g->ffn_ldd % VEC))))
            return false;
        if (g->ffn_mode == TC_FFN_LN_B && (!g->transA || g->transB || !(g->c_f32 || sizeof(T) == 4))) return false;
        if (g->ffn_mode == TC_FFN_EP && (g->transA || g->transB || g->c_f32 || g->accumulate || g->atomic || d.splitk != 1 || g->bias || g->R ||
                                         g->act != TC_ACT_NONE || (sizeof(T) == 2 && !d.vec8C) || (uintptr_t)g->ffn_d % 16 || g->ffn_ldd % VEC))
            return false;
    }
    return grid.y <= 65535 && grid.z <= 65535;
}

template <typename T>
int gemm_typed(const TcGemm* g, hipStream_t s) {
    GemmDev d;
    dim3 grid;
    bool use128;
    if (!gemm_plan<T>(g, d, grid, use128)) return TC_ERR_ARG;
    if (g->ffn_mode) return launch_ffn<T>(d, grid, s);
    if (g->c_f32)
        return use128 ? launch<T, float, 128, 128>(d, g->transA, g->transB, grid, s)
                      : launch<T, float, 64, 64>(d, g->transA, g->transB, grid, s);
    return use128 ? launch<T, T, 128, 128>(d, g->transA, g->transB, grid, s)
                  : launch<T, T, 64, 64>(d, g->transA, g->transB, grid, s);
}


}

static bool gemm_args_ok(const TcGemm* g) {
    if (!g || !g->A || !g->B || !g->C || g->M <= 0 || g->N <= 0 || g->K <= 0 || g->nb1 < 1 || g->nb2 < 1 || g->splitk < 1) return false;
    if ((g->splitk > 1 || g->atomic) && (!g->accumulate || (g->dtype != TC_F32 && !g->c_f32) || g->act != TC_ACT_NONE)) return false;
    if (g->act != TC_ACT_NONE && g->act != TC_ACT_SIGMOID && g->act != TC_ACT_SCALE) return false;
    if (g->act == TC_ACT_SCALE && g->ffn_mode != TC_FFN_NONE) return false;
    if (g->bgap_every < 0 || (g->bgap_every > 0 && (g->transB || g->bgap_every % 64 || (g->bgap % 8)))) return false;
    if (g->ffn_mode < TC_FFN_NONE || g->ffn_mode > TC_FFN_EP) return false;
    if (g->ffn_mode != TC_FFN_NONE) {
        if (!g->ffn_gamma || !g->ffn_beta || !g->ffn_stat || g->bgap_every) return false;
        if (g->ffn_mode == TC_FFN_LN_A && (!g->ffn_part || g->ffn_nchunk < 1 || g->ffn_chunk_n < 1)) return false;
        if (g->ffn_mode == TC_FFN_EP && (!g->ffn_d || !g->ffn_part2)) return false;
        if (g->ffn_sRow1 < 0 || g->ffn_sRow1 > 0x7fffffffLL || g->ffn_sPar1 < 0 || g->ffn_sPar1 > 0x7fffffffLL) return false;
    }
    return true;
}

#ifdef TC_GEMM_TIMING
extern "C" int tc_gemm_dbg_read(unsigned long long* dst, int reset) {
    int rc = (int)hipMemcpyFromSymbol(dst, HIP_SYMBOL(g_gemm_dbg), sizeof(unsigned long long) * 1024 * 8);
    if (reset) {
        static unsigned long long z[1024 * 8];
        unsigned int zn = 0;
        rc |= (int)hipMemcpyToSymbol(HIP_SYMBOL(g_gemm_dbg), z, sizeof(z));
        rc |= (int)hipMemcpyToSymbol(HIP_SYMBOL(g_gemm_dbg_n), &zn, sizeof(zn));
    }
    return rc;
}
#endif
extern "C" int tc_gemm(const TcGemm* g, void* stream) {
    if (!gemm_args_ok(g)) return TC_ERR_ARG;
    hipStream_t s = (hipStream_t)stream;
    TC_DISPATCH_DTYPE(g->dtype, return gemm_typed<T>(g, s));
    return TC_ERR_ARG;
}

extern "C" int tc_gemm_pair(const TcGemm* a, const TcGemm* b, void* stream) {
    if (!gemm_args_ok(a) || !gemm_args_ok(b) || a->bn_part || b->bn_part) return TC_ERR_ARG;
    hipStream_t s = (hipStream_t)stream;
    if ((a->dtype == TC_BF16 || a->dtype == TC_F16) && b->dtype == a->dtype && !a->transA && !a->transB && !a->c_f32 && b->transA && !b->transB && b->c_f32 &&
        (a->ffn_mode == TC_FFN_NONE || a->ffn_mode == TC_FFN_EP) && (b->ffn_mode == TC_FFN_NONE || b->ffn_mode == TC_FFN_LN_B)) {
        GemmPairDev q;
        dim3 ga, gb;
        bool bigA, bigB;
        if (!gemm_plan<bf16_t>(a, q.a, ga, bigA) || !gemm_plan<bf16_t>(b, q.b, gb, bigB)) return TC_ERR_ARG;
        const long long nA = (long long)ga.x * ga.y * ga.z, nB = (long long)gb.x * gb.y * gb.z;
        if (!bigA && !bigB && nA + nB < 0x7fffffffLL) {
            q.nA = (int)nA; q.gxA = ga.x; q.gyA = ga.y; q.gxB = gb.x; q.gyB = gb.y;
            q.mgxA = fdiv_make(ga.x, nA + nB); q.mgyA = fdiv_make(ga.y, nA + nB); q.mgxB = fdiv_make(gb.x, nA + nB); q.mgyB = fdiv_make(gb.y, nA + nB);
            if (gb.x * gb.y > 1) q.b.xcd |= 2;
            if (a->dtype == TC_BF16) hipLaunchKernelGGL(gemm_pair_kernel<bf16_t>, dim3((unsigned)(nA + nB)), dim3(256), 0, s, q);
            else hipLaunchKernelGGL(gemm_pair_kernel<f16_t>, dim3((unsigned)(nA + nB)), dim3(256), 0, s, q);
            return tc_launch_status();
        }
    }
    const int rc = tc_gemm(a, stream);
    return rc != TC_OK ? rc : tc_gemm(b, stream);
}

extern "C" int tc_gemm_multi(const TcGemm* g, int n, void* stream) {
    if (!g || n < 1) return TC_ERR_ARG;
    for (int i = 0; i < n; ++i) if (!gemm_args_ok(g + i) || g[i].bn_part) return TC_ERR_ARG;
    hipStream_t s = (hipStream_t)stream;
    bool ok = n <= GEMM_MULTI_MAX;
    GemmMultiDev q;
    GemmDev plan[GEMM_MULTI_MAX];
    dim3 grids[GEMM_MULTI_MAX];
    int kinds[GEMM_MULTI_MAX], order[GEMM_MULTI_MAX];
    for (int i = 0; ok && i < n; ++i) {
        const TcGemm& t = g[i];
        int kind = -1;
        const bool h16 = (t.dtype == TC_BF16 || t.dtype == TC_F16) && t.dtype == g[0].dtype;
        if (h16 && !t.transA && t.transB && !t.c_f32) kind = t.ffn_mode == TC_FFN_LN_A ? 3 : (t.ffn_mode ? -1 : 0);
        else if (h16 && !t.transA && !t.transB && !t.c_f32) kind = t.ffn_mode == TC_FFN_EP ? 4 : (t.ffn_mode ? -1 : 1);
        else if (h16 && t.transA && !t.transB && t.c_f32) kind = t.ffn_mode == TC_FFN_LN_B ? 5 : (t.ffn_mode ? -1 : 2);
        bool big;
        if (kind < 0 || !gemm_plan<bf16_t>(&t, plan[i], grids[i], big, true)) { ok = false; break; }
        kinds[i] = kind; order[i] = i;
    }
    long long blk = 0;
    if (ok) {
        std::stable_sort(order, order + n, [&](int a, int b) { return plan[a].kchunk > plan[b].kchunk; });
        for (int j = 0; j < n; ++j) {
            const int i = order[j];
            q.p[j] = plan[i]; q.kind[j] = kinds[i]; q.gx[j] = grids[i].x; q.gy[j] = grids[i].y; q.blk0[j] = (int)blk;
            q.mgy[j] = fdiv_make(grids[i].y, (unsigned long long)grids[i].x * grids[i].y * grids[i].z);
            if ((kinds[i] == 2 || kinds[i] == 5) && grids[i].x * grids[i].y > 1) q.p[j].xcd |= 2;
            blk += (long long)grids[i].x * grids[i].y * grids[i].z;
            if (blk > 0x7fffffffLL) ok = false;
        }
    }
    if (ok) {
        q.n = n;
        if (g[0].dtype == TC_BF16) hipLaunchKernelGGL(gemm_multi_kernel<bf16_t>, dim3((unsigned)blk), dim3(256), 0, s, q);
        else hipLaunchKernelGGL(gemm_multi_kernel<f16_t>, dim3((unsigned)blk), dim3(256), 0, s, q);
        return tc_launch_status();
    }
    for (int i = 0; i < n; ++i) {
        const int rc = tc_gemm(g + i, stream);
        if (rc != TC_OK) return rc;
    }
    return TC_OK;
}
```

### transception_amd/csrc/norm.hip

```cpp
#include "tc_common.h"
#include <cstdlib>

namespace {

constexpr int LN_MAXC = 2048;
#ifndef LN_FOLD
#define LN_FOLD 8
#endif
constexpr int LN_BWD_MAX_BLOCKS = 4096, LN_BWD_ROWS_PER_GROUP = 4;
constexpr int LN_BWD_WG_MIN = 1024;
inline int ln_bwd_blocks(bool deferred) {
    return deferred ? LN_BWD_MAX_BLOCKS : 1024;
}

struct LnMap { int p, H, W; };
__device__ __forceinline__ long long ln_row_off(int row, const LnMap& m, int ld, int C) {
    if (m.p == 0) return (long long)row * ld;
    const int Wp = m.W * m.p, Hp = m.H * m.p;
    const int ow = row % Wp, t = row / Wp, oh = t % Hp, b = t / Hp;
    return ((long long)(b * m.H + oh / m.p) * m.W + ow / m.p) * ld + ((oh % m.p) * m.p + ow % m.p) * C;
}

template <int GS> __device__ __forceinline__ float group_sum(float v) { return tc_group_sum<GS>(v); }

template <typename T, int GS, int NV, int RPT>
__global__ __launch_bounds__(256) void ln_fwd_kernel(const T* __restrict__ x, int ldx, const T* __restrict__ gamma,
                                                     const T* __restrict__ beta, T* __restrict__ y, int ldy,
                                                     float* __restrict__ mean, float* __restrict__ rstd, int rows,
                                                     int C, float eps, int act, long long pstride, LnMap map) {
    constexpr int RPB = 256 / GS;
    const int gl = threadIdx.x % GS, gi = threadIdx.x / GS;
    const int sst = (rstd == mean + 1) ? 2 : 1;
    {
        const long long g = blockIdx.y;
        x += g * rows * ldx; y += g * rows * ldy; mean += g * rows * sst; rstd += g * rows * sst; gamma += g * pstride; beta += g * pstride;
    }
    const int nv = C >> 2;
    const float invC = 1.0f / (float)C;
    float4 g[NV], b[NV];
#pragma unroll
    for (int i = 0; i < NV; ++i) {
        const int q = gl + i * GS;
        if (q < nv) { g[i] = ld4<T>(gamma + q * 4); b[i] = ld4<T>(beta + q * 4); }
    }
    for (int row0 = (blockIdx.x * RPB + gi) * RPT; row0 < rows; row0 += gridDim.x * RPB * RPT) {
        float4 v[RPT][NV];
        float mu[RPT], rs[RPT];
#pragma unroll
        for (int r = 0; r < RPT; ++r) {
            const int row = min(row0 + r, rows - 1);
            const T* xr = x + ln_row_off(row, map, ldx, C);
#pragma unroll
            for (int i = 0; i < NV; ++i) {
                const int q = gl + i * GS;
                v[r][i] = q < nv ? ld4<T>(xr + q * 4) : make_float4(0.f, 0.f, 0.f, 0.f);
            }
        }
#pragma unroll
        for (int r = 0; r < RPT; ++r) {
            float s = 0.f;
#pragma unroll
            for (int i = 0; i < NV; ++i) s += v[r][i].x + v[r][i].y + v[r][i].z + v[r][i].w;
            mu[r] = group_sum<GS>(s) * invC;
            float s2 = 0.f;
#pragma unroll
            for (int i = 0; i < NV; ++i) {
                const int q = gl + i * GS;
                if (q < nv) {
                    const float a = v[r][i].x - mu[r], bb = v[r][i].y - mu[r], c = v[r][i].z - mu[r], d = v[r][i].w - mu[r];
                    s2 += a * a + bb * bb + c * c + d * d;
                }
            }
            rs[r] = rsqrtf(group_sum<GS>(s2) * invC + eps);
        }
#pragma unroll
        for (int r = 0; r < RPT; ++r) {
            const int row = row0 + r;
            if (row >= rows) break;
            if (gl == 0) { mean[(long long)row * sst] = mu[r]; rstd[(long long)row * sst] = rs[r]; }
            T* yr = y + (long long)row * ldy;
#pragma unroll
            for (int i = 0; i < NV; ++i) {
                const int q = gl + i * GS;
                if (q < nv) {
                    float4 o;
                    o.x = (v[r][i].x - mu[r]) * rs[r] * g[i].x + b[i].x; o.y = (v[r][i].y - mu[r]) * rs[r] * g[i].y + b[i].y;
                    o.z = (v[r][i].z - mu[r]) * rs[r] * g[i].z + b[i].z; o.w = (v[r][i].w - mu[r]) * rs[r] * g[i].w + b[i].w;
                    if (act == TC_ACT_GELU) { o.x = gelu_fT<T>(o.x); o.y = gelu_fT<T>(o.y); o.z = gelu_fT<T>(o.z); o.w = gelu_fT<T>(o.w); }
                    st4<T>(yr + q * 4, o);
                }
            }
        }
    }
}

template <int RPB>
__device__ __forceinline__ void ln_bwd_param_tail(const float* red, const int C, float* __restrict__ dgamma, float* __restrict__ dbeta,
                                                  float* __restrict__ partial, int* __restrict__ cnt, const int defer) {
    __syncthreads();
    for (int c = threadIdx.x; c < C; c += 256) {
        float a = 0.f, bb = 0.f;
#pragma unroll
        for (int w = 0; w < RPB; ++w) { a += red[(w * 2 + 0) * C + c]; bb += red[(w * 2 + 1) * C + c]; }
        if (partial) {
// ... 816 lines not shown
```

### transception_amd/csrc/tc_common.h

```cpp
#pragma once
#include <hip/hip_runtime.h>
#include <type_traits>
#include <stdint.h>

#include "../../include/transception_hip.h"

typedef unsigned short bf16_t;

#define TC_WAVE 64

__device__ __forceinline__ float bf2f(bf16_t v) { return __uint_as_float(((unsigned)v) << 16); }
typedef float tc_f32x2 __attribute__((ext_vector_type(2)));
typedef __bf16 tc_bf16x2 __attribute__((ext_vector_type(2)));
__device__ __forceinline__ unsigned pack2bf(float lo, float hi) {
    const tc_f32x2 v = {lo, hi};
    return __builtin_bit_cast(unsigned, __builtin_convertvector(v, tc_bf16x2));
}
__device__ __forceinline__ bf16_t f2bf(float f) { return (bf16_t)(pack2bf(f, 0.f) & 0xffffu); }

struct f16_t { unsigned short v; };
typedef _Float16 tc_f16x2 __attribute__((ext_vector_type(2)));
__device__ __forceinline__ float h2f(f16_t v) { return (float)__builtin_bit_cast(_Float16, v.v); }
__device__ __forceinline__ unsigned pack2h(float lo, float hi) {
    const tc_f32x2 v = {lo, hi};
// ... 1 lines not shown
}
__device__ __forceinline__ f16_t f2h(float f) { f16_t r; r.v = __builtin_bit_cast(unsigned short, (_Float16)f); return r; }
template <typename T> __device__ __forceinline__ void unpack2(unsigned w, float& lo, float& hi);
template <> __device__ __forceinline__ void unpack2<bf16_t>(unsigned w, float& lo, float& hi) { lo = __uint_as_float(w << 16); hi = __uint_as_float(w & 0xffff0000u); }
template <> __device__ __forceinline__ void unpack2<f16_t>(unsigned w, float& lo, float& hi) {
    const tc_f16x2 h = __builtin_bit_cast(tc_f16x2, w);
    lo = (float)h.x; hi = (float)h.y;
}
template <typename T> __device__ __forceinline__ unsigned pack2(float lo, float hi);
template <> __device__ __forceinline__ unsigned pack2<bf16_t>(float lo, float hi) { return pack2bf(lo, hi); }
template <> __device__ __forceinline__ unsigned pack2<f16_t>(float lo, float hi) { return pack2h(lo, hi); }

typedef float tc_f32x16 __attribute__((ext_vector_type(16)));
typedef __bf16 tc_bf16x8 __attribute__((ext_vector_type(8)));
typedef _Float16 tc_f16x8 __attribute__((ext_vector_type(8)));
template <typename H> struct TcHalf;
template <> struct TcHalf<bf16_t> {
    typedef tc_bf16x8 v8; typedef __bf16 e;
    static __device__ __forceinline__ tc_f32x16 mfma(v8 a, v8 b, tc_f32x16 c) { return __builtin_amdgcn_mfma_f32_32x32x16_bf16(a, b, c, 0, 0, 0); }
};
template <> struct TcHalf<f16_t> {
    typedef tc_f16x8 v8; typedef _Float16 e;
    static __device__ __forceinline__ tc_f32x16 mfma(v8 a, v8 b, tc_f32x16 c) { return __builtin_amdgcn_mfma_f32_32x32x16_f16(a, b, c, 0, 0, 0); }
};

template <typename T> __device__ __forceinline__ float ldf(const T* p);
template <> __device__ __forceinline__ float ldf<float>(const float* p) { return *p; }
template <> __device__ __forceinline__ float ldf<bf16_t>(const bf16_t* p) { return bf2f(*p); }
template <> __device__ __forceinline__ float ldf<f16_t>(const f16_t* p) { return h2f(*p); }
template <typename T> __device__ __forceinline__ void stf(T* p, float v);
template <> __device__ __forceinline__ void stf<float>(float* p, float v) { *p = v; }
template <> __device__ __forceinline__ void stf<bf16_t>(bf16_t* p, float v) { *p = f2bf(v); }
template <> __device__ __forceinline__ void stf<f16_t>(f16_t* p, float v) { *p = f2h(v); }

template <typename T> __device__ __forceinline__ float4 ld4(const T* p);
template <> __device__ __forceinline__ float4 ld4<float>(const float* p) { return *reinterpret_cast<const float4*>(p); }
template <> __device__ __forceinline__ float4 ld4<bf16_t>(const bf16_t* p) {
    uint2 r = *reinterpret_cast<const uint2*>(p);
    return make_float4(__uint_as_float(r.x << 16), __uint_as_float(r.x & 0xffff0000u),
                       __uint_as_float(r.y << 16), __uint_as_float(r.y & 0xffff0000u));
}
template <> __device__ __forceinline__ float4 ld4<f16_t>(const f16_t* p) {
    const uint2 r = *reinterpret_cast<const uint2*>(p);
    float4 o;
    unpack2<f16_t>(r.x, o.x, o.y); unpack2<f16_t>(r.y, o.z, o.w);
    return o;
}
template <typename T> __device__ __forceinline__ void st4(T* p, float4 v);
template <> __device__ __forceinline__ void st4<float>(float* p, float4 v) { *reinterpret_cast<float4*>(p) = v; }
template <> __device__ __forceinline__ void st4<bf16_t>(bf16_t* p, float4 v) {
    uint2 r;
    r.x = pack2bf(v.x, v.y);
    r.y = pack2bf(v.z, v.w);
    *reinterpret_cast<uint2*>(p) = r;
}

template <> __device__ __forceinline__ void st4<f16_t>(f16_t* p, float4 v) {
    uint2 r;
    r.x = pack2h(v.x, v.y);
    r.y = pack2h(v.z, v.w);
    *reinterpret_cast<uint2*>(p) = r;
}

template <int CTRL> __device__ __forceinline__ float tc_dpp(float v) {
    return __builtin_bit_cast(float, __builtin_amdgcn_update_dpp(0, __builtin_bit_cast(int, v), CTRL, 0xf, 0xf, true));
}
template <int G> __device__ __forceinline__ float tc_group_sum(float v) {
    if (G >= 2) v += tc_dpp<0xB1>(v);
    if (G >= 4) v += tc_dpp<0x4E>(v);
    if (G >= 8) v += tc_dpp<0x141>(v);
    if (G >= 16) v += tc_dpp<0x140>(v);
    if (G >= 32) v += __shfl_xor(v, 16, 64);
    if (G >= 64) v += __shfl_xor(v, 32, 64);
    return v;
}
template <int G> __device__ __forceinline__ float tc_group_max(float v) {
    if (G >= 2) v = fmaxf(v, tc_dpp<0xB1>(v));
    if (G >= 4) v = fmaxf(v, tc_dpp<0x4E>(v));
    if (G >= 8) v = fmaxf(v, tc_dpp<0x141>(v));
    if (G >= 16) v = fmaxf(v, tc_dpp<0x140>(v));
    if (G >= 32) v = fmaxf(v, __shfl_xor(v, 16, 64));
    if (G >= 64) v = fmaxf(v, __shfl_xor(v, 32, 64));
    return v;
}

__device__ __forceinline__ int tc_mul24(int a, int b) { return a * b; }
__device__ __forceinline__ int tc_mad24(int a, int b, int c) { return a * b + c; }
struct SDiv { float inv, half; int d; };
__device__ __forceinline__ SDiv sdiv_make(int d) { SDiv s; s.inv = 1.0f / (float)d; s.half = 0.5f * s.inv; s.d = d; return s; }
__device__ __forceinline__ int sdiv(int n, const SDiv& s) { return (int)fmaf((float)n, s.inv, s.half); }
__device__ __forceinline__ int smod(int n, int q, const SDiv& s) { return n - q * s.d; }
__device__ __forceinline__ int tc_opaque(int v) { asm volatile("" : "+v"(v)); return v; }
__device__ __forceinline__ float wave_sum(float v) { return tc_group_sum<64>(v); }
__device__ __forceinline__ float wave_max(float v) { return tc_group_max<64>(v); }

template <bool FAST> __device__ __forceinline__ float tc_rcp(float x) { return FAST ? __builtin_amdgcn_rcpf(x) : __frcp_rn(x); }
template <bool FAST = false> __device__ __forceinline__ float gelu_cdf_pdf(float x, float& pdf) {
    const float z = fabsf(x) * 0.70710678118654752440f;
    const float g = __expf(-z * z);
    const float t = tc_rcp<FAST>(fmaf(0.3275911f, z, 1.0f));
    float poly = fmaf(1.061405429f, t, -1.453152027f);
    poly = fmaf(poly, t, 1.421413741f);
    poly = fmaf(poly, t, -0.284496736f);
    poly = fmaf(poly, t, 0.254829592f);
    const float half_erfc = 0.5f * poly * t * g;
    pdf = 0.39894228040143267794f * g;
    return x >= 0.f ? 1.0f - half_erfc : half_erfc;
}
__device__ __forceinline__ float gelu_f(float x) { float pdf; return x * gelu_cdf_pdf(x, pdf); }
template <typename T> __device__ __forceinline__ float gelu_grad_fT(float x) {
    float pdf;
    const float cdf = gelu_cdf_pdf<!std::is_same<T, float>::value>(x, pdf);
    return cdf + x * pdf;
}
template <typename T> __device__ __forceinline__ float sigmoid_fT(float x) { return tc_rcp<!std::is_same<T, float>::value>(1.0f + __expf(-x)); }
__device__ __forceinline__ tc_f32x2 gelu_cdf_pdf2(tc_f32x2 x, tc_f32x2& pdf) {
    const tc_f32x2 ax = {fabsf(x.x), fabsf(x.y)};
    const tc_f32x2 z = ax * 0.70710678118654752440f;
    const tc_f32x2 nz2 = -z * z;
    const tc_f32x2 g = {__expf(nz2.x), __expf(nz2.y)};
    const tc_f32x2 den = z * 0.3275911f + 1.0f;
    const tc_f32x2 t = {__frcp_rn(den.x), __frcp_rn(den.y)};
    tc_f32x2 poly = t * 1.061405429f + (-1.453152027f);
    poly = poly * t + 1.421413741f;
    poly = poly * t + (-0.284496736f);
    poly = poly * t + 0.254829592f;
    const tc_f32x2 half_erfc = poly * t * g * 0.5f;
    pdf = g * 0.39894228040143267794f;
    const tc_f32x2 one_m = 1.0f - half_erfc;
    return tc_f32x2{x.x >= 0.f ? one_m.x : half_erfc.x, x.y >= 0.f ? one_m.y : half_erfc.y};
}
__device__ __forceinline__ tc_f32x2 gelu_cdf_pdf2_fast(tc_f32x2 x, tc_f32x2& pdf) {
    const tc_f32x2 ax = {fabsf(x.x), fabsf(x.y)};
    const tc_f32x2 z = ax * 0.70710678118654752440f;
    const tc_f32x2 nz2 = -z * z;
    const tc_f32x2 g = {__expf(nz2.x), __expf(nz2.y)};
    const tc_f32x2 den = z * 0.3275911f + 1.0f;
    const tc_f32x2 t = {__builtin_amdgcn_rcpf(den.x), __builtin_amdgcn_rcpf(den.y)};
    tc_f32x2 poly = t * 1.061405429f + (-1.453152027f);
    poly = poly * t + 1.421413741f;
    poly = poly * t + (-0.284496736f);
    poly = poly * t + 0.254829592f;
    const tc_f32x2 half_erfc = poly * t * g * 0.5f;
    pdf = g * 0.39894228040143267794f;
    const tc_f32x2 one_m = 1.0f - half_erfc;
    return tc_f32x2{x.x >= 0.f ? one_m.x : half_erfc.x, x.y >= 0.f ? one_m.y : half_erfc.y};
}
__device__ __forceinline__ tc_f32x2 gelu_f2_fast(tc_f32x2 x) { tc_f32x2 pdf; return x * gelu_cdf_pdf2_fast(x, pdf); }
#define TC_PHI_X0 4.2f
#define TC_PHI_C0 3.9890743800e-01f
#define TC_PHI_C1 -6.6360416413e-02f
#define TC_PHI_C2 9.8301434219e-03f
#define TC_PHI_C3 -1.1141502210e-03f
#define TC_PHI_C4 9.4574729576e-05f
#define TC_PHI_C5 -5.7608060352e-06f
#define TC_PHI_C6 2.3436991163e-07f
#define TC_PHI_C7 -5.6334089611e-09f
#define TC_PHI_C8 5.9982045543e-11f
__device__ __forceinline__ float gelu_poly(float x) {
    const float t = __builtin_amdgcn_fmed3f(x, -TC_PHI_X0, TC_PHI_X0), s = t * t;
    float p = fmaf(TC_PHI_C8, s, TC_PHI_C7);
    p = fmaf(p, s, TC_PHI_C6); p = fmaf(p, s, TC_PHI_C5); p = fmaf(p, s, TC_PHI_C4); p = fmaf(p, s, TC_PHI_C3);
    p = fmaf(p, s, TC_PHI_C2); p = fmaf(p, s, TC_PHI_C1); p = fmaf(p, s, TC_PHI_C0);
    return x * fmaf(t, p, 0.5f);
}
__device__ __forceinline__ tc_f32x2 gelu_poly2(tc_f32x2 x) {
// ... 74 lines not shown
```

### transception_amd/engine.py

```python
from __future__ import annotations

import ctypes as C
import os
from typing import Callable, Dict, List, Optional, Tuple

import torch

from ._lib import (ATTN_DKV_SPLITS, EW_COPY, EW_DEINTERLEAVE, EW_PATCHIFY, TcEffAtt, TcEwSeg, TcFfnBwd, TcFfnFused, ACT_COORD, ACT_GELU, ACT_HSWISH, ACT_NONE, ACT_SCALE, ACT_SIGMOID, FFN_EP, FFN_LN_A, FFN_LN_B, TC_BF16, TC_F16, TC_F32, TcDwSeg, TcFfnSeg,
                   TcGemm, lib)

_DT = {torch.float32: TC_F32, torch.bfloat16: TC_BF16, torch.float16: TC_F16}

PROFILE: Optional[dict] = None


SEG_MARKS = os.environ.get("TC_SEG_MARKS", "")
SEG_LABELS: List[str] = []


def _timed(name: str, flops: float, fn):
    if PROFILE is None:
        fn()
        return
    e0, e1 = torch.cuda.Event(enable_timing=True), torch.cuda.Event(enable_timing=True)
    e0.record()
    fn()
    e1.record()
    PROFILE.setdefault(name, []).append((e0, e1, flops))


def _gemm_work(descs):
    fl = by = 0.0
    for g in descs:
        nb = g.nb1 * g.nb2
        es = 4 if g.dtype == TC_F32 else 2
        ec = 4 if g.c_f32 else es
        fl += 2.0 * g.M * g.N * g.K * nb
        by += nb * ((g.M * g.K + g.K * g.N) * es + g.M * g.N * ec * (2 if g.accumulate else 1) + (g.M * g.N * es if g.R else 0))
    return fl, by


def _timed_gemm(kind: str, descs, fn):
    if PROFILE is None:
        fn()
        return
    _timed("gemm:" + kind, _gemm_work(descs), fn)


class P:
    __slots__ = ("data", "grad", "gs")

    def __init__(self, data: torch.Tensor, grad: Optional[torch.Tensor], gs: int = 0):
        self.data = data
        self.grad = grad
        self.gs = gs


class Var:
    __slots__ = ("data", "root", "path", "kids", "grad_t", "whole_written", "written", "requires_grad", "region", "reshaped", "covered", "bn_part")

    def __init__(self, data: torch.Tensor, root: "Var" = None, path=None, requires_grad: bool = True, region=None,
                 reshaped: bool = False):
        assert data.dim() == 2 and (data.stride(1) == 1 or data.shape[1] == 1), (data.shape, data.stride())
        self.data = data
        self.root = root if root is not None else self
        self.path = path or ()
        self.kids: Dict[tuple, Var] = {}
        self.grad_t: Optional[torch.Tensor] = None
        self.whole_written = False
        self.written: List[tuple] = []
        self.requires_grad = requires_grad
        self.region = region if region is not None else (0, data.shape[0], 0, data.shape[1])
        self.covered = False
        self.reshaped = reshaped

    rows = property(lambda s: s.data.shape[0])
    cols = property(lambda s: s.data.shape[1])
    ld = property(lambda s: s.data.stride(0))

    def _kid(self, key, data, region, reshaped=False):
        k = self.kids.get(key)
        if k is None:
            k = Var(data, self.root, self.path + (key,), self.root.requires_grad, region, reshaped)
            self.kids[key] = k
        return k

    def colslice(self, a: int, b: int) -> "Var":
        assert not self.reshaped, "slice before reshaping"
        r0, r1, c0, _ = self.region
        return self._kid(("c", a, b), self.data[:, a:b], (r0, r1, c0 + a, c0 + b))

    def rowslice(self, a: int, b: int) -> "Var":
        assert not self.reshaped, "slice before reshaping"
        r0, _, c0, c1 = self.region
        return self._kid(("r", a, b), self.data[a:b], (r0 + a, r0 + b, c0, c1))

    def reshape(self, rows: int, cols: int) -> "Var":
        assert self.data.is_contiguous() and self.region[2] == 0 and self.region[3] == self.root.data.shape[1]
        return self._kid(("v", rows, cols), self.data.view(rows, cols), self.region, True)

    @property
    def is_whole(self) -> bool:
        rt = self.root.data
        return self.region == (0, rt.shape[0], 0, rt.shape[1])

    def apply_path(self, t: torch.Tensor) -> torch.Tensor:
        for k in self.path:
            if k[0] == "c":
                t = t[:, k[1]:k[2]]
            elif k[0] == "r":
                t = t[k[1]:k[2]]
            else:
                t = t.view(k[1], k[2])
        return t


def _overlap(a, b) -> bool:
    return a[0] < b[1] and b[0] < a[1] and a[2] < b[3] and b[2] < a[3]


def _ptr(t: Optional[torch.Tensor]):
    return None if t is None else t.data_ptr()


_WORKSPACES: Dict[Tuple[str, str], torch.Tensor] = {}
WORKSPACE_BYTES = 16384 + 1024 * 16384


def _workspace(device, tag: str = "") -> torch.Tensor:
    key = (str(device), tag)
    ws = _WORKSPACES.get(key)
    if ws is None:
        ws = _WORKSPACES[key] = torch.zeros(WORKSPACE_BYTES * (8 if tag == "many" else 1), dtype=torch.uint8, device=device)
    return ws


_SPLITK_CAP = 128
_SPLITK_BLOCKS = 512
_SPLITK_KMIN = 384
_THR128 = 100000
_FFN_STORE_ACT = os.environ.get("TC_FFN_STORE_ACT", "1") != "0"
_FFN_LN_GEMM_MAXC = int(os.environ.get("TC_FFN_LN_GEMM_MAXC", "64"))
_FFN_TILED = os.environ.get("TC_FFN_TILED", "1") != "0"
_DW_DEFER = os.environ.get("TC_DW_DEFER", "1") != "0"
_LN_DEFER = os.environ.get("TC_LN_DEFER", "1") != "0"
_EFFATT_FUSED = os.environ.get("TC_EFFATT_FUSED", "1") != "0"
_FFN_PRE_LN = os.environ.get("TC_FFN_PRE_LN", "0") != "0"
_LIN_LN_FUSED = os.environ.get("TC_LIN_LN_FUSED", "1") != "0"
_RIPM_FUSED = os.environ.get("TC_RIPM_FUSED", "1") != "0"
_LN_CLS_FUSED = os.environ.get("TC_LN_CLS_FUSED", "1") != "0"
_DW_LN_FUSED = os.environ.get("TC_DW_LN_FUSED", "1") != "0"
_MHCA_ATT_BWD_FUSED = os.environ.get("TC_MHCA_ATT_BWD_FUSED", "1") != "0"
_MHCA_ATT_FUSED = os.environ.get("TC_MHCA_ATT_FUSED", "1") != "0"
_DW_BWD_ONE = os.environ.get("TC_DW_BWD_ONE", "1") != "0"
_FFN_TILED_BWD = os.environ.get("TC_FFN_TILED_BWD", "1") != "0"
_FFN_TILE_BWD = (0, 0)
_FFN_TILE = (0, 0)
# ... 149 lines not shown
    def segment(self, name: str):
        if not SEG_MARKS:
            return
        prev = self._seg_prev
        self._seg_prev = name
        SEG_LABELS.append("F:" + name)
        self.L.tc_seg_marker(len(SEG_LABELS) - 1, self.stream)

        def bwd():
            SEG_LABELS.append("B:" + (prev or "head"))
            self.L.tc_seg_marker(len(SEG_LABELS) - 1, self.stream)
        self._rec(bwd)

    def backward(self, until: Optional[str] = None) -> bool:
        while self.tape:
            entry = self.tape.pop()
            if callable(entry):
                entry()
            elif entry[1] == until:
                self._flush_param_folds()
                return False
        self._flush_param_folds()
        self.tape = []
        self._zeros.close()
        if SEG_MARKS:
            import json
            with open(SEG_MARKS, "w") as f:
                json.dump(SEG_LABELS, f)
        return True

    def _flush_dw_folds(self):
        from ._lib import TcDwFold
        for c0 in range(0, len(self._dw_pending), 48):
            chunk = self._dw_pending[c0:c0 + 48]
            arr = (TcDwFold * len(chunk))(*[site for site, _ in chunk])
            self.n_launch += 1
            self.L.tc_dw_fold(arr, len(chunk), self.stream)
        self._dw_pending = []

    def _flush_param_folds(self):
        self._flush_dw_folds()
        if not self._ln_pending:
            return
        from ._lib import TcLnFold
        arr = (TcLnFold * len(self._ln_pending))()
        for i, (part, dg, db, gs, nblk, Cc, Gn) in enumerate(self._ln_pending):
            arr[i].part, arr[i].dgamma, arr[i].dbeta, arr[i].pstride = _ptr(part), _ptr(dg), _ptr(db), gs
            arr[i].nblk, arr[i].C, arr[i].groups = nblk, Cc, Gn
        self.n_launch += 1
        self.L.tc_layernorm_fold(arr, len(self._ln_pending), self.stream)
        self._ln_pending = []

    def _rec(self, fn):
        if self.record:
            self.tape.append(fn)

    def _gemm(self, A, lda, B, ldb, Cm, ldc, M, N, K, tA, tB, bias=None, R=None, ldr=0, alpha=1.0, acc=0, act=ACT_NONE,
              splitk=1, nb1=1, nb2=1, sA=(0, 0), sB=(0, 0), sC=(0, 0), sR=(0, 0), c_f32=0, atomic=0, rowsum=None, sbias=0, srow=0,
              bn_part=None, bn_shift=None):
        g = self._gemm_desc(A, lda, B, ldb, Cm, ldc, M, N, K, tA, tB, bias, R, ldr, alpha, acc, act, splitk, nb1, nb2, sA, sB, sC, sR,
                            c_f32, atomic, rowsum, sbias, srow)
        if bn_part is not None:
            g.bn_part, g.bn_shift = bn_part, bn_shift
        self.n_launch += 1
        _timed_gemm("single", [g], lambda: self.L.tc_gemm(C.byref(g), self.stream))

    def _gemm_desc(self, A, lda, B, ldb, Cm, ldc, M, N, K, tA, tB, bias=None, R=None, ldr=0, alpha=1.0, acc=0, act=ACT_NONE,
                   splitk=1, nb1=1, nb2=1, sA=(0, 0), sB=(0, 0), sC=(0, 0), sR=(0, 0), c_f32=0, atomic=0, rowsum=None, sbias=0,
                   srow=0, use_ws=True, bgap=(0, 0)) -> TcGemm:
        ws = _workspace(self.dev) if use_ws else None
        return TcGemm(A, B, Cm, bias, R, M, N, K, lda, ldb, ldc, ldr, tA, tB, nb1, nb2, sA[0], sA[1], sB[0], sB[1], sC[0], sC[1],
                      sR[0], sR[1], alpha, acc, act, splitk, self.dt, c_f32, atomic, rowsum, sbias, srow, bgap[0], bgap[1],
                      ws.data_ptr() if ws is not None else None, ws.numel() if ws is not None else 0)

    @staticmethod
    def _small_tiles(m_out: int, n_out: int, nb: int) -> bool:
        return ((m_out + 127) // 128) * ((n_out + 127) // 128) * nb < _THR128 or m_out < 96 or n_out < 96

    @staticmethod
    def _splitk(m_out: int, n_out: int, k_red: int) -> int:
        tiles = ((m_out + 63) // 64) * ((n_out + 63) // 64)
        cap = _SPLITK_CAP if k_red < 262144 else 1024
        return max(1, min(max(_SPLITK_BLOCKS, cap) // max(tiles, 1), k_red // _SPLITK_KMIN, cap))

    def linear(self, x: Var, W: P, b: Optional[P] = None, out: Optional[Var] = None, residual: Optional[Var] = None,
               act: int = ACT_NONE, wcols: Optional[Tuple[int, int]] = None, accumulate: bool = False,
               batch: Optional[Tuple[int, int, int, int]] = None, post_scale: Optional[float] = None,
               bn_shift: Optional[torch.Tensor] = None, launch: bool = True) -> Var:
        Wt = W.data if wcols is None else W.data[:, wcols[0]:wcols[1]]
        N, K = Wt.shape
        assert x.cols == K, (x.cols, K)
        Gn = self.ngroups
        grouped = Gn > 1
        M = x.rows // Gn
        if out is None:
            assert batch is None
            out = self.new(x.rows, N)
        if grouped:
            assert batch is None and W.gs > 0 and (b is None or b.gs == W.gs)
            side_by_side = (out.rows == M and out.cols == Gn * N)
            assert side_by_side or (out.rows == Gn * M and out.cols == N)
            nb, sx, so, sr = Gn, M * x.ld, (N if side_by_side else M * out.ld), (M * residual.ld if residual is not None else 0)
            sw = W.gs
        else:
            side_by_side = False
            assert out.rows == M and out.cols == N
            nb, sx, so, sr = batch if batch is not None else (1, 0, 0, 0)
            sw = 0
        if post_scale is not None:
            assert act == ACT_NONE and not accumulate
        bn_part = None
        if (bn_shift is not None and self.training and self.dtype != torch.float32 and nb == 1 and not accumulate
                and act == ACT_NONE and post_scale is None and N % 8 == 0 and out.ld % 8 == 0 and out.data.data_ptr() % 16 == 0):
            tiles = (M + 63) // 64
            bn_part = self.f32(N * (1 + 2 * max(tiles, 128)))
            out.bn_part = (bn_part, tiles)
        if launch:
            self._gemm(_ptr(x.data), x.ld, _ptr(Wt), Wt.stride(0), _ptr(out.data), out.ld, M, N, K, 0, 1,
                       bias=_ptr(b.data) if b is not None else None, R=_ptr(residual.data) if residual is not None else None,
                       ldr=residual.ld if residual is not None else 0, acc=int(accumulate), act=act if post_scale is None else ACT_SCALE,
                       alpha=1.0 if post_scale is None else post_scale, nb1=nb, sA=(sx, 0), sB=(sw, 0), sC=(so, 0), sR=(sr, 0), sbias=sw,
                       bn_part=_ptr(bn_part) if bn_part is not None else None, bn_shift=_ptr(bn_shift) if bn_part is not None else None)

        def bwd():
            dy = self.grad_of(out)
            if dy is None:
                return
            dz = dy
            if act == ACT_SIGMOID:
                assert dy.is_contiguous() and out.data.is_contiguous() and (nb == 1 or (grouped and not side_by_side))
                dz = torch.empty_like(dy)
                self.L.tc_sigmoid_bwd(_ptr(dy), _ptr(out.data), _ptr(dz), dy.numel(), self.dt, self.stream)
            want_db = b is not None and b.grad is not None
            paired = (x.requires_grad and W.grad is not None and self.dtype != torch.float32
                      and self._small_tiles(M, K, nb) and self._small_tiles(N, K, nb))
            if paired:
                gx, acc = self.wgrad(x, (nb - 1) * sx // x.root.cols if (nb > 1 and not grouped) else 0)
                gW = W.grad if wcols is None else W.grad[:, wcols[0]:wcols[1]]
                ga = self._gemm_desc(_ptr(dz), dz.stride(0), _ptr(Wt), Wt.stride(0), _ptr(gx), gx.stride(0), M, K, N, 0, 0, acc=acc,
                                     nb1=nb, sA=(so, 0), sB=(sw, 0), sC=(sx, 0))
                gb = self._gemm_desc(_ptr(dz), dz.stride(0), _ptr(x.data), x.ld, _ptr(gW), gW.stride(0), N, K, M, 1, 0, acc=1,
                                     splitk=self._splitk(N, K, M), c_f32=1, nb1=nb, sA=(so, 0), sB=(sx, 0), sC=(sw, 0),
                                     atomic=int(nb > 1 and not grouped), rowsum=_ptr(b.grad) if want_db else None, srow=sw,
                                     use_ws=False)
                if gb.splitk > 128:
                    gb.ws, gb.ws_bytes, ga.ws, ga.ws_bytes = ga.ws, ga.ws_bytes, None, 0
                self.n_launch += 1
                _timed_gemm("pair", [ga, gb], lambda: self.L.tc_gemm_pair(C.byref(ga), C.byref(gb), self.stream))
            elif x.requires_grad:
                gx, acc = self.wgrad(x, (nb - 1) * sx // x.root.cols if (nb > 1 and not grouped) else 0)
                self._gemm(_ptr(dz), dz.stride(0), _ptr(Wt), Wt.stride(0), _ptr(gx), gx.stride(0), M, K, N, 0, 0, acc=acc,
                           nb1=nb, sA=(so, 0), sB=(sw, 0), sC=(sx, 0))
            if paired:
                pass
            elif W.grad is not None:
                gW = W.grad if wcols is None else W.grad[:, wcols[0]:wcols[1]]
                self._gemm(_ptr(dz), dz.stride(0), _ptr(x.data), x.ld, _ptr(gW), gW.stride(0), N, K, M, 1, 0, acc=1,
                           splitk=self._splitk(N, K, M), c_f32=1, nb1=nb, sA=(so, 0), sB=(sx, 0), sC=(sw, 0),
                           atomic=int(nb > 1 and not grouped), rowsum=_ptr(b.grad) if want_db else None, srow=sw)
            elif want_db:
                assert not grouped
                self.L.tc_colsum(_ptr(dz), M, N, dz.stride(0), nb, so, _ptr(b.grad), 1, self.dt, self.stream)
            if residual is not None:
                if nb == 1 or (grouped and not side_by_side):
                    self.pass_grad(residual, dy)
                else:
                    assert grouped or sr == so
                    self._pass_grad_batched(residual, dy, nb, M, N, so, sr if grouped else so)
        self._rec(bwd)
        return out

    def linear_many(self, items: List[tuple]) -> List[Var]:
        n = len(items)
        assert self.ngroups == 1 and n >= 1
        items = [tuple(it) + (None,) * (7 - len(it)) for it in items]
        wsb = _workspace(self.dev, "many")
        sl = (wsb.numel() // 8) & ~16383

        def desc(i, *a, **k):
            g = self._gemm_desc(*a, use_ws=False, **k)
            if i < 8:
                g.ws, g.ws_bytes = wsb.data_ptr() + i * sl, sl
            return g

        def launch(probs):
            for c0 in range(0, len(probs), 12):
                chunk = probs[c0:c0 + 12]
                arr = (TcGemm * len(chunk))(*chunk)
                self.n_launch += 1
                _timed_gemm("multi", chunk, lambda: self.L.tc_gemm_multi(arr, len(chunk), self.stream))
        fw = []
        for i, (x, W, b, out, res, batch, ps) in enumerate(items):
            N, K = W.data.shape
            nb, sx, so, sr = batch if batch is not None else (1, 0, 0, 0)
            assert x.cols == K and out.rows == x.rows and out.cols == N
            fw.append(desc(i % 12, _ptr(x.data), x.ld, _ptr(W.data), W.data.stride(0), _ptr(out.data), out.ld, x.rows, N, K, 0, 1,
                           bias=_ptr(b.data) if b is not None else None, R=_ptr(res.data) if res is not None else None,
                           ldr=res.ld if res is not None else 0, nb1=nb, sA=(sx, 0), sC=(so, 0), sR=(sr, 0),
                           alpha=1.0 if ps is None else ps, act=ACT_NONE if ps is None else ACT_SCALE))
        launch(fw)

        def bwd():
            dxs, dws = [], []
            waves: List[list] = []
            for i, (x, W, b, out, res, batch, _ps) in enumerate(items):
                dy = self.grad_of(out)
                if dy is None:
                    continue
                N, K = W.data.shape
                M = x.rows
                nb, sx, so, sr = batch if batch is not None else (1, 0, 0, 0)
                if x.requires_grad:
                    ext = (nb - 1) * sx // x.root.cols if nb > 1 else 0
                    gx, acc = self.wgrad(x, ext)
                    reg = (id(x.root), (x.region[0], x.region[1] + ext, x.region[2], x.region[3]))
                    wi = 0
                    while wi < len(waves) and any(r[0] == reg[0] and _overlap(r[1], reg[1]) for r, _ in waves[wi]):
                        wi += 1
                    if wi == len(waves):
                        waves.append([])
                    waves[wi].append((reg, desc(len(waves[wi]) % 8, _ptr(dy), dy.stride(0), _ptr(W.data), W.data.stride(0), _ptr(gx),
                                                gx.stride(0), M, K, N, 0, 0, acc=acc, nb1=nb, sA=(so, 0), sC=(sx, 0))))
                if W.grad is not None:
                    dws.append(self._gemm_desc(_ptr(dy), dy.stride(0), _ptr(x.data), x.ld, _ptr(W.grad), W.grad.stride(0), N, K, M, 1, 0,
                                               acc=1, splitk=self._splitk(N, K, M), c_f32=1, nb1=nb, sA=(so, 0), sB=(sx, 0),
                                               atomic=1,
                                               rowsum=_ptr(b.grad) if (b is not None and b.grad is not None) else None,
                                               use_ws=False))
                if res is not None:
                    if nb == 1:
                        self.pass_grad(res, dy)
                    else:
# ... 274 lines not shown
                                   acc=1, splitk=self._splitk(t["C4"], t["Cin"], t["M"]), c_f32=1, nb1=Gn, sA=(t["M"] * t["C4"], 0),
                                   sB=(t["M"] * x.ld, 0), sC=(gs, 0), rowsum=_ptr(t["b1"].grad) if t["b1"].grad is not None else None, srow=gs,
                                   use_ws=False))
            self._launch_gemms(g2)
            for t in st:
                for k in ("gp", "part2", "dh"):
                    t.pop(k, None)
        self._rec(bwd)
        return [t["out"] for t in st_all]

    def _pass_grad_batched(self, v: Var, src: torch.Tensor, nb: int, M: int, N: int, sb_src: int, sb_dst: Optional[int] = None,
                           defer: bool = False):
        sb_dst = sb_src if sb_dst is None else sb_dst
        g, acc = self.wgrad(v, 0 if v.rows >= nb * M else (nb - 1) * sb_dst // v.root.cols)
        if defer:
            return TcEwSeg(EW_COPY, acc, src.data_ptr(), g.data_ptr(), sb_src, sb_dst, src.stride(0), g.stride(0), nb, M, N, 0, 0, 0)
        self.L.tc_copy3d(_ptr(src), sb_src, src.stride(0), _ptr(g), sb_dst, g.stride(0), nb, M, N, acc, self.dt, self.stream)

    def effatt_supported(self, t: Var, params: Optional[Tuple[P, ...]] = None) -> bool:
        if self.record and (not t.requires_grad or (params is not None and any(p.grad is None for p in params))):
            return False
        return (_EFFATT_FUSED and self.ngroups == 1 and self.dt != TC_F32
                and bool(self.L.tc_effatt_supported(t.cols, self.dt)) and t.data.is_contiguous())

    def eff_attention_block(self, t: Var, ln: Tuple[P, P], keys: Tuple[P, P], queries: Tuple[P, P], values: Tuple[P, P],
                            reproj: Tuple[P, P], B: int, N: int, eps: float = 1e-5) -> Var:
        L, Cc = self.L, t.cols
        assert t.rows == B * N and self.effatt_supported(t)
        out = self.new(t.rows, Cc)
        nf = int(L.tc_effatt_scratch_floats(Cc, B, N))
        ctx, kstat = self.f32(B, Cc, Cc), self.f32(B, 2, Cc)
        es = t.data.element_size()

        def desc(part, dout=None, dt=None, g1=None, acc=0, grads=False):
            f = TcEffAtt()
            f.t, f.gamma, f.beta = _ptr(t.data), _ptr(ln[0].data), _ptr(ln[1].data)
            for nm, (W, b) in (("k", keys), ("q", queries), ("v", values), ("r", reproj)):
                setattr(f, "w" + nm, _ptr(W.data)); setattr(f, "b" + nm, _ptr(b.data))
                if grads:
                    setattr(f, "dw" + nm, _ptr(W.grad)); setattr(f, "db" + nm, _ptr(b.grad))
            if grads:
                f.dgamma, f.dbeta = _ptr(ln[0].grad), _ptr(ln[1].grad)
            f.out, f.ctx, f.kstat, f.part, f.part_floats = _ptr(out.data), _ptr(ctx), _ptr(kstat), _ptr(part), nf
            f.ldt, f.ldo, f.C, f.B, f.N, f.eps = t.ld, out.ld, Cc, B, N, eps
            if dout is not None:
                f.dout, f.lddo, f.dt, f.lddt, f.g1, f.acc_dt = _ptr(dout), dout.stride(0), _ptr(dt), dt.stride(0), _ptr(g1), acc
            return f

        part = self.f32(nf)
        f = desc(part)
        self.n_launch += 3
        _timed("hbm:effatt_fwd (LayerNorm + EfficientAttention + residual: token statistics, context fold, output)",
               3.0 * t.rows * Cc * es, lambda: L.tc_effatt_fwd(C.byref(f), self.dt, self.stream))
        del part

        def bwd():
            dy = self.grad_of(out)
            if dy is None or not t.requires_grad:
                return
            gx, acc = self.wgrad(t)
            part = self.f32(nf)
            g1 = _empty((t.rows, Cc), self.dtype, self.dev)
            fb = desc(part, dy, gx, g1, acc, grads=True)
            self.n_launch += 4
            _timed("hbm:effatt_bwd (query side + d_ctx partials, d_ctx fold, key/value side + LayerNorm backward, parameter fold)",
                   (6.0 + acc) * t.rows * Cc * es, lambda: L.tc_effatt_bwd(C.byref(fb), self.dt, self.stream))
        self._rec(bwd)
        return out

    def layernorm(self, x: Var, g: P, b: P, eps: float = 1e-5, act: int = ACT_NONE, out: Optional[Var] = None,
                  stats: Optional[Tuple[torch.Tensor, torch.Tensor]] = None, launch: bool = True) -> Var:
        Gn = self.ngroups
        rows, Cc = x.rows // Gn, x.cols
        assert Gn == 1 or (g.gs > 0 and b.gs == g.gs)
        if out is None:
            out = self.new(x.rows, Cc)
        mean, rstd = stats if stats is not None else (self.f32(x.rows), self.f32(x.rows))
        es = x.data.element_size()
        if launch:
            _timed("hbm:layernorm_fwd", 2.0 * x.rows * Cc * es, lambda: self.L.tc_layernorm_fwd(
                _ptr(x.data), x.ld, _ptr(g.data), _ptr(b.data), _ptr(out.data), out.ld, _ptr(mean), _ptr(rstd), rows, Cc, eps, act, Gn, g.gs,
                self.dt, self.stream))

        def bwd():
            dy = self.grad_of(out)
            if dy is None or not x.requires_grad:
                return
            gx, acc = self.wgrad(x)
            fused = g.grad is not None
            nblk = int(self.L.tc_layernorm_bwd_nblk(rows, Cc)) if (fused and _LN_DEFER) else 0
            if nblk > 0:
                nf = Gn * nblk * 2 * Cc
                part = self.f32(nf)
                _timed("hbm:layernorm_bwd", (3.0 + acc) * x.rows * Cc * es, lambda: self.L.tc_layernorm_bwd_defer(
                    _ptr(dy), dy.stride(0), _ptr(x.data), x.ld, _ptr(g.data), _ptr(b.data), _ptr(mean), _ptr(rstd), _ptr(gx), gx.stride(0),
                    _ptr(gx) if acc else None, gx.stride(0), _ptr(g.grad), _ptr(b.grad), rows, Cc, act, Gn, g.gs, _ptr(part), nf, self.dt,
                    self.stream))
                self._ln_pending.append((part, g.grad, b.grad, g.gs, nblk, Cc, Gn))
                if len(self._ln_pending) == 64:
                    self._flush_param_folds()
                return
            if fused:
                ws = _workspace(self.dev)
                scratch, n = ws, ws.numel() // 4
                _timed("hbm:layernorm_bwd", (3.0 + acc) * x.rows * Cc * es, lambda: self.L.tc_layernorm_bwd(
                    _ptr(dy), dy.stride(0), _ptr(x.data), x.ld, _ptr(g.data), _ptr(b.data), _ptr(mean), _ptr(rstd), _ptr(gx), gx.stride(0),
                    _ptr(gx) if acc else None, gx.stride(0), _ptr(g.grad), _ptr(b.grad), rows, Cc, act, Gn, g.gs, _ptr(scratch), n, self.dt,
                    self.stream))
                return
            self.L.tc_layernorm_bwd(_ptr(dy), dy.stride(0), _ptr(x.data), x.ld, _ptr(g.data), _ptr(b.data), _ptr(mean),
                                    _ptr(rstd), _ptr(gx), gx.stride(0), _ptr(gx) if acc else None, gx.stride(0),
                                    None, None, rows, Cc, act, Gn, g.gs, None, 0, self.dt, self.stream)
        self._rec(bwd)
        return out

    def layernorm_shuffled(self, x: Var, g: P, b: P, B: int, H: int, W: int, p: int, eps: float = 1e-5) -> Var:
        assert self.ngroups == 1 and x.rows == B * H * W and x.cols % (p * p) == 0
        c = x.cols // (p * p)
        rows = B * H * p * W * p
        out = self.new(rows, c)
        mean, rstd = self.f32(rows), self.f32(rows)
        es = x.data.element_size()
        _timed("hbm:layernorm_fwd", 2.0 * rows * c * es, lambda: self.L.tc_layernorm_ps_fwd(
            _ptr(x.data), x.ld, _ptr(g.data), _ptr(b.data), _ptr(out.data), out.ld, _ptr(mean), _ptr(rstd), B, H, W, p, c, eps, self.dt,
            self.stream))

        def bwd():
            dy = self.grad_of(out)
            if dy is None or not x.requires_grad:
                return
            gx, acc = self.wgrad(x)
            assert not acc, "the expanded map has one consumer"
            ws = _workspace(self.dev)
            _timed("hbm:layernorm_bwd", 3.0 * rows * c * es, lambda: self.L.tc_layernorm_ps_bwd(
                _ptr(dy), dy.stride(0), _ptr(x.data), x.ld, _ptr(g.data), _ptr(b.data), _ptr(mean), _ptr(rstd), _ptr(gx), gx.stride(0),
                _ptr(g.grad), _ptr(b.grad), B, H, W, p, c, _ptr(ws) if g.grad is not None else None, ws.numel() // 4, self.dt, self.stream))
        self._rec(bwd)
        return out

    def ln_cls_supported(self, x: Var, p: int, g: P, b: P, Wc: P, bc: Optional[P], B: int = 0, H: int = 0, W: int = 0) -> bool:
        c = x.cols // max(p * p, 1)
        if p >= 2 and B * H * p * W * p * max(H, W) * p >= 1 << 32:
            return False
        return (_LN_CLS_FUSED and self.dt != TC_F32 and self.ngroups == 1 and bc is not None and x.ld % 8 == 0
                and all(q.data.data_ptr() % 16 == 0 for q in (x, g, b, Wc)) and Wc.data.is_contiguous() and Wc.data.shape[1] == c
                and bool(self.L.tc_ln_cls_supported(c, Wc.data.shape[0], self.dt)))

    def ln_cls(self, x: Var, g: P, b: P, Wc: P, bc: P, B: int, H: int, W: int, p: int, eps: float = 1e-5, pad_rows: bool = False) -> Var:
        assert self.ngroups == 1 and x.rows == B * H * W and x.cols % max(p * p, 1) == 0
        c = x.cols // max(p * p, 1)
        ncls = Wc.data.shape[0]
        rows = B * H * p * W * p if p else x.rows
        out = self.new(rows, (ncls + 7) // 8 * 8).colslice(0, ncls) if pad_rows else self.new(rows, ncls)
        mean, rstd = self.f32(rows), self.f32(rows)
        es = x.data.element_size()
        self.n_launch += 1
        _timed("hbm:ln_cls_fwd (pixel shuffle + LayerNorm + classifier, one launch)", 1.0 * rows * (c + ncls) * es, lambda: self.L.tc_ln_cls_fwd(
            _ptr(x.data), x.ld, _ptr(g.data), _ptr(b.data), _ptr(Wc.data), _ptr(bc.data), _ptr(out.data), out.ld, _ptr(mean), _ptr(rstd),
            B, H, W, p, c, ncls, eps, self.dt, self.stream))

        def bwd():
            dl = self.grad_of(out)
            if dl is None or not x.requires_grad:
                return
            gx, acc = self.wgrad(x)
            assert not acc, "the expanded map has one consumer"
# ... 939 lines not shown
```

Measured before the change: 1462 images/sec.

## Fuse LayerNorm backward into the epilogue of the following linear's dX GEMM

When a LayerNorm output feeds exactly one linear layer, the dX GEMM of that linear now runs the LayerNorm backward in its epilogue. The full-row dY tile is staged in LDS, and the row sums, dX and the per-block gamma/beta partials are computed there. This removes the separate LayerNorm backward kernel and one round trip of the intermediate gradient through HBM. The cost is forcing 64-row tiles with whole 64- or 128-wide rows, no split-K on that GEMM, and more epilogue work and LDS use, which may lower occupancy. It also adds new pair and multi kernel variants.

```diff
diff --git a/include/transception_hip.h b/include/transception_hip.h
--- a/include/transception_hip.h
+++ b/include/transception_hip.h
@@ -46,6 +46,18 @@
 int tc_gemm(const TcGemm* g, void* stream);
 int tc_gemm_pair(const TcGemm* a, const TcGemm* b, void* stream);
 int tc_gemm_multi(const TcGemm* g, int n, void* stream);
+
+typedef struct {
+    const void* x; const void* dres; const void* gamma;
+    const float* mean; const float* rstd;
+    float* part; long long part_floats;
+    long long pstride;
+    int ldx, ldres, map_p, map_H, map_W, reserved;
+} TcGemmLn;
+int tc_gemm_ln_supported(int C, int dtype);
+int tc_gemm_ln(const TcGemm* g, const TcGemmLn* ln, void* stream);
+int tc_gemm_pair_ln(const TcGemm* a, const TcGemmLn* ln, const TcGemm* b, void* stream);
+int tc_gemm_multi_ln(const TcGemm* g, const TcGemmLn* ln, int n, void* stream);
 
 int tc_colsum(const void* x, int rows, int cols, int ldx, int nb, long long sb, float* out, int accumulate, int dtype,
               void* stream);
diff --git a/transception_amd/_lib.py b/transception_amd/_lib.py
--- a/transception_amd/_lib.py
+++ b/transception_amd/_lib.py
@@ -32,6 +32,11 @@
 FFN_NONE, FFN_LN_A, FFN_LN_B, FFN_EP = 0, 1, 2, 3
 
 
+class TcGemmLn(C.Structure):
+    _fields_ = [("x", vp), ("dres", vp), ("gamma", vp), ("mean", vp), ("rstd", vp), ("part", vp), ("part_floats", i64), ("pstride", i64),
+                ("ldx", i32), ("ldres", i32), ("map_p", i32), ("map_H", i32), ("map_W", i32), ("reserved", i32)]
+
+
 class TcDwSeg(C.Structure):
     _fields_ = [("x", vp), ("w", vp), ("bias", vp), ("y", vp), ("dy", vp), ("dw", vp), ("db", vp), ("C", i32), ("k", i32),
                 ("ldx", i32), ("ldy", i32), ("lddy", i32), ("B", i32), ("H", i32), ("W", i32), ("stat", vp)]
@@ -105,6 +110,10 @@
     "tc_ew_multi": [C.POINTER(TcEwSeg), i32, i32, vp],
     "tc_gemm_pair": [C.POINTER(TcGemm), C.POINTER(TcGemm), vp],
     "tc_gemm_multi": [C.POINTER(TcGemm), i32, vp],
+    "tc_gemm_ln_supported": [i32, i32],
+    "tc_gemm_ln": [C.POINTER(TcGemm), C.POINTER(TcGemmLn), vp],
+    "tc_gemm_pair_ln": [C.POINTER(TcGemm), C.POINTER(TcGemmLn), C.POINTER(TcGemm), vp],
+    "tc_gemm_multi_ln": [C.POINTER(TcGemm), C.POINTER(TcGemmLn), i32, vp],
     "tc_colsum": [vp, i32, i32, i32, i32, i64, vp, i32, i32, vp],
     "tc_layernorm_fwd": [vp, i32, vp, vp, vp, i32, vp, vp, i32, i32, f32, i32, i32, i64, i32, vp],
     "tc_layernorm_bwd": [vp, i32, vp, i32, vp, vp, vp, vp, vp, i32, vp, i32, vp, vp, i32, i32, i32, i32, i64, vp, i64, i32, vp],
@@ -239,7 +248,7 @@
     "tc_mhca_att_fwd": [vp, i32, vp, vp, vp, vp, vp, vp, vp, vp, i64, vp, i32, vp, i32, vp, i32, vp, i32, i32, i32, i32, i32, f32, i32, vp],
 }
 _RET = {"tc_ln_cls_scratch_floats": i64, "tc_ffn_fused_bwd_scratch_floats": i64, "tc_effatt_scratch_floats": i64, "tc_bn_scratch_floats": i64, "tc_softmax_scratch_floats": i64, "tc_layernorm_bwd_scratch_floats": i64, "tc_dwconv_bwd_plan": i64, "tc_dwconv_multi_plan": i64, "tc_ffn_mid_plan": i64, "tc_factor_att_stats_floats": i64, "tc_metric_hist_bins": i64}
-_RAW = {"tc_abi_version", "tc_ln_cls_supported", "tc_ln_cls_scratch_floats", "tc_linear_ln_supported", "tc_ripm_supported", "tc_ripm_tiles", "tc_mhca_att_supported", "tc_dw_ln_supported", "tc_mhca_att_bwd_supported", "tc_effatt_supported", "tc_effatt_scratch_floats", "tc_ffn_chunk", "tc_ffn_fused_supported", "tc_ffn_fused_bwd_supported", "tc_ffn_fused_bwd_scratch_floats", "tc_bn_scratch_floats", "tc_softmax_scratch_floats", "tc_layernorm_bwd_scratch_floats", "tc_layernorm_bwd_nblk", "tc_dwconv_bwd_plan", "tc_dwconv_multi_plan", "tc_ffn_mid_plan", "tc_factor_att_stats_floats", "tc_metric_hist_bins"}
+_RAW = {"tc_abi_version", "tc_gemm_ln_supported", "tc_ln_cls_supported", "tc_ln_cls_scratch_floats", "tc_linear_ln_supported", "tc_ripm_supported", "tc_ripm_tiles", "tc_mhca_att_supported", "tc_dw_ln_supported", "tc_mhca_att_bwd_supported", "tc_effatt_supported", "tc_effatt_scratch_floats", "tc_ffn_chunk", "tc_ffn_fused_supported", "tc_ffn_fused_bwd_supported", "tc_ffn_fused_bwd_scratch_floats", "tc_bn_scratch_floats", "tc_softmax_scratch_floats", "tc_layernorm_bwd_scratch_floats", "tc_layernorm_bwd_nblk", "tc_dwconv_bwd_plan", "tc_dwconv_multi_plan", "tc_ffn_mid_plan", "tc_factor_att_stats_floats", "tc_metric_hist_bins"}
 
 
 class TcError(RuntimeError):
diff --git a/transception_amd/csrc/gemm.hip b/transception_amd/csrc/gemm.hip
--- a/transception_amd/csrc/gemm.hip
+++ b/transception_amd/csrc/gemm.hip
@@ -47,6 +47,7 @@
     __device__ __host__ const float* bn_shift() const { return ffn.part; }
 };
 constexpr int GEMM_BN_STATS = 4;
+constexpr int GEMM_LN_BWD = 5;
 
 template <typename H> __device__ __forceinline__ void bf8_unpack(const uint4& r, float* o) {
     unpack2<H>(r.x, o[0], o[1]); unpack2<H>(r.y, o[2], o[3]); unpack2<H>(r.z, o[4], o[5]); unpack2<H>(r.w, o[6], o[7]);
@@ -430,6 +431,99 @@
     }
 }
 
+template <typename H, int BM, int BN, int TM, int TN>
+__device__ __forceinline__ void epilogue_rows_lds_lnbwd(const GemmDev& p, f32x16 (&acc)[TM][TN], int b1, int m0, int wr, int wc, int lane,
+                                                        bf16_t* stage_raw, int by, int gy) {
+    constexpr int LDS_ = BN + 8, WM = BM / 2, WN = BN / 2, C = BN, GS = BN / 8, RPB = 256 / GS, NIT = BM / RPB;
+    static_assert(BM % RPB == 0 && GS <= 16, "a lane group stays inside one DPP row");
+    H* stage = reinterpret_cast<H*>(stage_raw);
+    float* red = reinterpret_cast<float*>(stage_raw + BM * LDS_);
+    const int tid = threadIdx.x, gl = tid % GS, gi = tid / GS, h = lane >> 5;
+    const LnMap map{p.ffn.nchunk, p.ffn.chunk_n, p.ffn.sRow1};
+    const int ldx = p.ffn.ldd;
+    const H* x = reinterpret_cast<const H*>(p.ffn.d) + (long long)b1 * p.M * ldx;
+    const H* dres = p.R ? reinterpret_cast<const H*>(p.R) + (long long)b1 * p.M * p.ldr : nullptr;
+    H* dx = reinterpret_cast<H*>(p.C) + b1 * p.sC1;
+    const float* mean = p.ffn.part + (long long)b1 * p.M;
+    const float* rstd = p.ffn.stat + (long long)b1 * p.M;
+    const bool has_res = dres != nullptr, has_par = p.ffn.part2 != nullptr;
+    uint4 rx[NIT], rr[NIT];
+    float mu[NIT], rs[NIT], g[8], ag[8], ab[8];
+#pragma unroll
+    for (int it = 0; it < NIT; ++it) {
+        const int row = min(m0 + gi + it * RPB, p.M - 1);
+        rx[it] = *reinterpret_cast<const uint4*>(x + ln_row_off(row, map, ldx, C) + gl * 8);
+        if (has_res) rr[it] = *reinterpret_cast<const uint4*>(dres + ln_row_off(row, map, p.ldr, C) + gl * 8);
+        mu[it] = mean[row]; rs[it] = rstd[row];
+    }
+    bf8_unpack<H>(*reinterpret_cast<const uint4*>(reinterpret_cast<const H*>(p.ffn.gamma) + (long long)b1 * p.ffn.sPar1 + gl * 8), g);
+#pragma unroll
+    for (int j = 0; j < 8; ++j) ag[j] = ab[j] = 0.f;
+    __syncthreads();
+#pragma unroll
+    for (int i = 0; i < TM; ++i) {
+        const int lr = wr * WM + i * 32 + (lane & 31);
+#pragma unroll
+        for (int j = 0; j < TN; ++j)
+#pragma unroll
+            for (int q = 0; q < 4; ++q) {
+                const int lc = wc * WN + j * 32 + 8 * q + 4 * h;
+                st4<H>(stage + lr * LDS_ + lc, make_float4(p.alpha * acc[i][j][4 * q], p.alpha * acc[i][j][4 * q + 1], p.alpha * acc[i][j][4 * q + 2],
+                                                           p.alpha * acc[i][j][4 * q + 3]));
+            }
+    }
+    __syncthreads();
+    constexpr float invC = 1.0f / (float)C;
+#pragma unroll
+    for (int it = 0; it < NIT; ++it) {
+        const int lr = gi + it * RPB;
+        const bool live = m0 + lr < p.M;
+        float xv[8], d[8];
+        bf8_unpack<H>(rx[it], xv);
+        bf8_unpack<H>(*reinterpret_cast<const uint4*>(stage + lr * LDS_ + gl * 8), d);
+#pragma unroll
+        for (int j = 0; j < 8; ++j) xv[j] = (xv[j] - mu[it]) * rs[it];
+        if (has_par && live) {
+#pragma unroll
+            for (int j = 0; j < 8; ++j) { ag[j] += d[j] * xv[j]; ab[j] += d[j]; }
+        }
+#pragma unroll
+        for (int j = 0; j < 8; ++j) d[j] *= g[j];
+        float s1 = ((d[0] + d[1]) + d[2]) + d[3]; s1 += ((d[4] + d[5]) + d[6]) + d[7];
+        float s2 = ((d[0] * xv[0] + d[1] * xv[1]) + d[2] * xv[2]) + d[3] * xv[3]; s2 += ((d[4] * xv[4] + d[5] * xv[5]) + d[6] * xv[6]) + d[7] * xv[7];
+        s1 = tc_group_sum<GS>(s1) * invC; s2 = tc_group_sum<GS>(s2) * invC;
+        if (!live) continue;
+        float o[8];
+#pragma unroll
+        for (int j = 0; j < 8; ++j) o[j] = rs[it] * (d[j] - s1 - xv[j] * s2);
+        if (has_res) {
+            float q[8];
+            bf8_unpack<H>(rr[it], q);
+#pragma unroll
+            for (int j = 0; j < 8; ++j) o[j] += q[j];
+        }
+        *reinterpret_cast<uint4*>(dx + ln_row_off(m0 + lr, map, p.ldc, C) + gl * 8) = bf8_pack<H>(o);
+    }
+    if (!has_par) return;
+#pragma unroll
+    for (int j = 0; j < 8; ++j)
+#pragma unroll
+        for (int o = GS; o < 64; o <<= 1) { ag[j] += __shfl_xor(ag[j], o, 64); ab[j] += __shfl_xor(ab[j], o, 64); }
+    if (lane < GS) {
+        const int wave = tid >> 6;
+#pragma unroll
+        for (int j = 0; j < 8; ++j) { red[(wave * 2 + 0) * C + gl * 8 + j] = ag[j]; red[(wave * 2 + 1) * C + gl * 8 + j] = ab[j]; }
+    }
+    __syncthreads();
+    float* pp = p.ffn.part2 + ((long long)b1 * gy + by) * 2 * C;
+    for (int c = tid; c < C; c += 256) {
+        float a = 0.f, bb = 0.f;
+#pragma unroll
+        for (int w = 0; w < 4; ++w) { a += red[(w * 2 + 0) * C + c]; bb += red[(w * 2 + 1) * C + c]; }
+        pp[c] = a; pp[C + c] = bb;
+    }
+}
+
 __device__ __forceinline__ float4 load_strip(const float* base, int ld, int x, int k, int X, int K, bool trans, bool vec) {
     float4 v = make_float4(0.f, 0.f, 0.f, 0.f);
     if (!trans) {
@@ -656,7 +750,8 @@
 __device__ __forceinline__ void gemm_bf16_body(const GemmDev& p, const int bx, const int by, const int bz, const int gx, const int gy,
                                                bf16_t (*As)[BM * (64 + 8)], bf16_t (*Bs)[BN * (64 + 8)]) {
     constexpr int BK = 64, LDT = BK + 8;
-    static_assert(FFN == 0 || (BM == 64 && BN == 64 && DB), "the MixFFN hooks run on 64x64 tiles with the double-buffered LDS");
+    static_assert(FFN == 0 || FFN == GEMM_LN_BWD || (BM == 64 && BN == 64 && DB), "the MixFFN hooks run on 64x64 tiles with the double-buffered LDS");
+    static_assert(FFN != GEMM_LN_BWD || (BM == 64 && (BN == 64 || BN == 128) && DB && !TA && !TB && sizeof(TC) == 2), "LayerNorm backward: whole 64- / 128-wide rows of a dX product");
     static_assert(FFN != TC_FFN_LN_A || !TA, "LN_A transforms rows of a row-major A");
     static_assert(FFN != TC_FFN_LN_B || !TB, "LN_B transforms rows of a [K,N] B");
     static_assert(FFN != TC_FFN_EP || sizeof(TC) == 2, "EP writes a bf16 C");
@@ -867,7 +962,10 @@
         if (!splitk_fixup<TM, TN>(p, acc, (zq * gy + by) * gx + bx, ks, grp)) return;
         first = (grp == 0); atomic = p.fix_ngroups > 1;
     }
-    if constexpr (FFN == TC_FFN_EP) {
+    if constexpr (FFN == GEMM_LN_BWD) {
+        static_assert(FFN != GEMM_LN_BWD || BM * (BN + 8) + 4 * 2 * BN * 2 <= 2 * (BM + BN) * (64 + 8), "C stage + parameter-gradient sums must fit");
+        epilogue_rows_lds_lnbwd<H, BM, BN, TM, TN>(p, acc, b1, m0, wr, wc, lane, &As[0][0], by, gy);
+    } else if constexpr (FFN == TC_FFN_EP) {
         static_assert(FFN != TC_FFN_EP || 2 * BM * (BN + 8) + 2 * BM * 4 <= 2 * (BM + BN) * (64 + 8), "C stage + d tile + row sums must fit");
         epilogue_rows_lds_ep<H, BM, BN, TM, TN>(p, acc, b1, m0, n0, wr, wc, lane, &As[0][0], rd0, rd1, bx, gx);
     } else if constexpr (SWAP) {
@@ -905,9 +1003,9 @@
 }
 
 struct GemmPairDev { GemmDev a, b; int nA, gxA, gyA, gxB, gyB; unsigned mgxA, mgyA, mgxB, mgyB; };
-template <typename H>
-__global__ __launch_bounds__(256, 2) void gemm_pair_kernel(GemmPairDev q) {
-    __shared__ __attribute__((aligned(16))) bf16_t smem[2 * (64 + 64) * (64 + 8)];
+template <typename H, int LNW>
+__device__ __forceinline__ void gemm_pair_body(const GemmPairDev& q, bf16_t* smem) {
+    constexpr int BNA = LNW ? LNW : 64;
     bf16_t(*As)[64 * (64 + 8)] = reinterpret_cast<bf16_t(*)[64 * (64 + 8)]>(smem);
     bf16_t(*Bs)[64 * (64 + 8)] = reinterpret_cast<bf16_t(*)[64 * (64 + 8)]>(smem + 2 * 64 * (64 + 8));
     const int nB = (int)gridDim.x - q.nA;
@@ -918,7 +1016,10 @@
         const int bz = fdiv(l1, q.gyA, q.mgyA);
         int by = l1 - bz * q.gyA;
         if (q.a.xcd & 1) tc_xcd_tile(bx, by, q.gxA, q.gyA, q.mgxA);
-        if (q.a.ffn.mode == TC_FFN_EP) gemm_bf16_body<H, H, 64, 64, false, false, true, TC_FFN_EP>(q.a, bx, by, bz, q.gxA, q.gyA, As, Bs);
+        if constexpr (LNW != 0)
+            gemm_bf16_body<H, H, 64, BNA, false, false, true, GEMM_LN_BWD>(q.a, bx, by, bz, q.gxA, q.gyA, As,
+                                                                          reinterpret_cast<bf16_t(*)[BNA * (64 + 8)]>(smem + 2 * 64 * (64 + 8)));
+        else if (q.a.ffn.mode == TC_FFN_EP) gemm_bf16_body<H, H, 64, 64, false, false, true, TC_FFN_EP>(q.a, bx, by, bz, q.gxA, q.gyA, As, Bs);
         else gemm_bf16_body<H, H, 64, 64, false, false, true>(q.a, bx, by, bz, q.gxA, q.gyA, As, Bs);
     } else {
         lin -= q.nA;
@@ -930,6 +1031,16 @@
         if (q.b.ffn.mode == TC_FFN_LN_B) gemm_bf16_body<H, float, 64, 64, true, false, true, TC_FFN_LN_B>(q.b, bx, by, bz, q.gxB, q.gyB, As, Bs);
         else gemm_bf16_body<H, float, 64, 64, true, false, true>(q.b, bx, by, bz, q.gxB, q.gyB, As, Bs);
     }
+}
+template <typename H>
+__global__ __launch_bounds__(256, 2) void gemm_pair_kernel(GemmPairDev q) {
+    __shared__ __attribute__((aligned(16))) bf16_t smem[2 * (64 + 64) * (64 + 8)];
+    gemm_pair_body<H, 0>(q, smem);
+}
+template <typename H, int LNW>
+__global__ __launch_bounds__(256, 2) void gemm_pair_ln_kernel(GemmPairDev q) {
+    __shared__ __attribute__((aligned(16))) bf16_t smem[2 * (64 + LNW) * (64 + 8)];
+    gemm_pair_body<H, LNW>(q, smem);
 }
 
 constexpr int GEMM_MULTI_MAX = 12;
@@ -959,6 +1070,7 @@
     else if (q.kind[i] == 2) gemm_bf16_body<H, float, 64, 64, true, false, true>(p, bx, by, bz, gx, gy, As, Bs);
     else if (q.kind[i] == 3) gemm_bf16_body<H, H, 64, 64, false, true, true, TC_FFN_LN_A>(p, bx, by, bz, gx, gy, As, Bs);
     else if (q.kind[i] == 4) gemm_bf16_body<H, H, 64, 64, false, false, true, TC_FFN_EP>(p, bx, by, bz, gx, gy, As, Bs);
+    else if (q.kind[i] == 6) gemm_bf16_body<H, H, 64, 64, false, false, true, GEMM_LN_BWD>(p, bx, by, bz, gx, gy, As, Bs);
     else gemm_bf16_body<H, float, 64, 64, true, false, true, TC_FFN_LN_B>(p, bx, by, bz, gx, gy, As, Bs);
 }
 
@@ -983,6 +1095,17 @@
     return tc_launch_status();
 }
 
+template <typename T>
+int launch_lnbwd(const GemmDev& d, dim3 grid, hipStream_t s) {
+    if constexpr (sizeof(T) == 2) {
+        if (d.N == 64) hipLaunchKernelGGL((gemm_bf16_kernel<T, T, 64, 64, false, false, true, GEMM_LN_BWD>), grid, dim3(256), 0, s, d);
+        else hipLaunchKernelGGL((gemm_bf16_kernel<T, T, 64, 128, false, false, true, GEMM_LN_BWD>), grid, dim3(256), 0, s, d);
+        return tc_launch_status();
+    } else {
+        return TC_ERR_ARG;
+    }
+}
+
 template <typename T, typename TC, int BM, int BN>
 int launch(const GemmDev& d, int transA, int transB, dim3 grid, hipStream_t s) {
     if (!transA && transB) launch_one<T, TC, BM, BN, false, true>(d, grid, s);
@@ -993,7 +1116,7 @@
 }
 
 template <typename T>
-bool gemm_plan(const TcGemm* g, GemmDev& d, dim3& grid, bool& use128_out, bool force64 = false) {
+bool gemm_plan(const TcGemm* g, GemmDev& d, dim3& grid, bool& use128_out, bool force64 = false, const TcGemmLn* ln = nullptr) {
     d.A = g->A; d.B = g->B; d.C = g->C; d.bias = g->bias; d.R = g->R;
     d.M = g->M; d.N = g->N; d.K = g->K; d.lda = g->lda; d.ldb = g->ldb; d.ldc = g->ldc; d.ldr = g->ldr;
     d.nb2 = g->nb2; d.splitk = g->splitk;
@@ -1009,7 +1132,7 @@
     d.ffn.d = g->ffn_mode == TC_FFN_LN_A ? g->ffn_aout : g->ffn_d;
     d.ffn.part2 = g->ffn_part2;
     if (g->bn_part && !g->ffn_mode) { d.ffn.mode = GEMM_BN_STATS; d.ffn.part2 = g->bn_part; d.ffn.part = g->bn_shift; }
-    if (g->ffn_mode || g->bn_part) force64 = true;
+    if (g->ffn_mode || g->bn_part || ln) force64 = true;
     constexpr int VEC = 16 / (int)sizeof(T);
     auto aligned = [&](const void* ptr, int ld, long long s1, long long s2) {
         return ((uintptr_t)ptr % 16 == 0) && (ld % VEC == 0) && (s1 % VEC == 0) && (s2 % VEC == 0);
@@ -1041,7 +1164,7 @@
 #define GEMM_AS_TARGET 512
 #define GEMM_AS_KPER 256
 #endif
-        if (want == 1 && !g->atomic && g->ffn_mode != TC_FFN_EP && !g->bn_part && g->K >= 2 * GEMM_AS_KPER && tiles64 <= GEMM_AS_TILES) {
+        if (want == 1 && !g->atomic && g->ffn_mode != TC_FFN_EP && !g->bn_part && !ln && g->K >= 2 * GEMM_AS_KPER && tiles64 <= GEMM_AS_TILES) {
             long long sk = GEMM_AS_TARGET / tiles64;
             if (sk > g->K / GEMM_AS_KPER) sk = g->K / GEMM_AS_KPER;
             if (sk > FIX_GROUP) sk = FIX_GROUP;
@@ -1084,15 +1207,35 @@
                                          g->act != TC_ACT_NONE || (sizeof(T) == 2 && !d.vec8C) || (uintptr_t)g->ffn_d % 16 || g->ffn_ldd % VEC))
             return false;
     }
+    if (ln) {
+        const long long prow = (long long)ln->map_p * ln->map_p * g->N;
+        if (sizeof(T) != 2 || (g->N != 64 && g->N != 128) || g->ffn_mode || g->bn_part || g->transA || g->transB || g->c_f32 || g->accumulate ||
+            g->atomic || g->splitk != 1 || d.splitk != 1 || g->bias || g->R || g->act != TC_ACT_NONE || g->nb2 != 1 || !d.vec8C ||
+            !ln->x || !ln->gamma || !ln->mean || !ln->rstd || (uintptr_t)ln->x % 16 || ln->ldx % 8 || (uintptr_t)ln->gamma % 16 || ln->pstride % 8 ||
+            (ln->dres && ((uintptr_t)ln->dres % 16 || ln->ldres % 8)) || ln->map_p < 0 ||
+            (g->nb1 > 1 && (ln->map_p || g->sC1 != (long long)g->M * g->ldc || ln->pstride <= 0 || ln->pstride > 0x7fffffffLL)) ||
+            (ln->map_p && (ln->map_H < 1 || ln->map_W < 1 || g->M % ((long long)ln->map_H * ln->map_W * ln->map_p * ln->map_p) || ln->ldx < prow ||
+                           g->ldc < prow || (ln->dres && ln->ldres < prow))) ||
+            (!ln->map_p && (ln->ldx < g->N || (ln->dres && ln->ldres < g->N))))
+            return false;
+        grid = dim3(1, (g->M + 63) / 64, nb);
+        if (ln->part && ln->part_floats < (long long)nb * grid.y * 2 * g->N) return false;
+        d.xcd = 0;
+        d.ffn.mode = GEMM_LN_BWD; d.ffn.d = ln->x; d.ffn.ldd = ln->ldx; d.R = ln->dres; d.ldr = ln->ldres;
+        d.ffn.part = ln->mean; d.ffn.stat = const_cast<float*>(ln->rstd); d.ffn.gamma = ln->gamma; d.ffn.beta = nullptr; d.ffn.part2 = ln->part;
+        d.ffn.sPar1 = g->nb1 > 1 ? (int)ln->pstride : 0;
+        d.ffn.nchunk = ln->map_p; d.ffn.chunk_n = ln->map_H; d.ffn.sRow1 = ln->map_W;
+    }
     return grid.y <= 65535 && grid.z <= 65535;
 }
 
 template <typename T>
-int gemm_typed(const TcGemm* g, hipStream_t s) {
+int gemm_typed(const TcGemm* g, hipStream_t s, const TcGemmLn* ln = nullptr) {
     GemmDev d;
     dim3 grid;
     bool use128;
-    if (!gemm_plan<T>(g, d, grid, use128)) return TC_ERR_ARG;
+    if (!gemm_plan<T>(g, d, grid, use128, false, ln)) return TC_ERR_ARG;
+    if (ln) return launch_lnbwd<T>(d, grid, s);
     if (g->ffn_mode) return launch_ffn<T>(d, grid, s);
     if (g->c_f32)
         return use128 ? launch<T, float, 128, 128>(d, g->transA, g->transB, grid, s)
@@ -1139,32 +1282,69 @@
     return TC_ERR_ARG;
 }
 
-extern "C" int tc_gemm_pair(const TcGemm* a, const TcGemm* b, void* stream) {
-    if (!gemm_args_ok(a) || !gemm_args_ok(b) || a->bn_part || b->bn_part) return TC_ERR_ARG;
+static bool gemm_ln_args_ok(const TcGemm* g, const TcGemmLn* ln) {
+    return ln && (g->dtype == TC_BF16 || g->dtype == TC_F16) && tc_gemm_ln_supported(g->N, g->dtype);
+}
+
+static int gemm_pair_impl(const TcGemm* a, const TcGemmLn* ln, const TcGemm* b, void* stream) {
+    if (!gemm_args_ok(a) || !gemm_args_ok(b) || a->bn_part || b->bn_part || (ln && !gemm_ln_args_ok(a, ln))) return TC_ERR_ARG;
     hipStream_t s = (hipStream_t)stream;
     if ((a->dtype == TC_BF16 || a->dtype == TC_F16) && b->dtype == a->dtype && !a->transA && !a->transB && !a->c_f32 && b->transA && !b->transB && b->c_f32 &&
         (a->ffn_mode == TC_FFN_NONE || a->ffn_mode == TC_FFN_EP) && (b->ffn_mode == TC_FFN_NONE || b->ffn_mode == TC_FFN_LN_B)) {
         GemmPairDev q;
         dim3 ga, gb;
         bool bigA, bigB;
-        if (!gemm_plan<bf16_t>(a, q.a, ga, bigA) || !gemm_plan<bf16_t>(b, q.b, gb, bigB)) return TC_ERR_ARG;
+        if (!gemm_plan<bf16_t>(a, q.a, ga, bigA, false, ln) || !gemm_plan<bf16_t>(b, q.b, gb, bigB)) return TC_ERR_ARG;
         const long long nA = (long long)ga.x * ga.y * ga.z, nB = (long long)gb.x * gb.y * gb.z;
         if (!bigA && !bigB && nA + nB < 0x7fffffffLL) {
             q.nA = (int)nA; q.gxA = ga.x; q.gyA = ga.y; q.gxB = gb.x; q.gyB = gb.y;
             q.mgxA = fdiv_make(ga.x, nA + nB); q.mgyA = fdiv_make(ga.y, nA + nB); q.mgxB = fdiv_make(gb.x, nA + nB); q.mgyB = fdiv_make(gb.y, nA + nB);
             if (gb.x * gb.y > 1) q.b.xcd |= 2;
-            if (a->dtype == TC_BF16) hipLaunchKernelGGL(gemm_pair_kernel<bf16_t>, dim3((unsigned)(nA + nB)), dim3(256), 0, s, q);
-            else hipLaunchKernelGGL(gemm_pair_kernel<f16_t>, dim3((unsigned)(nA + nB)), dim3(256), 0, s, q);
+            const dim3 grid((unsigned)(nA + nB));
+            const bool bf = a->dtype == TC_BF16;
+            if (!ln) {
+                if (bf) hipLaunchKernelGGL(gemm_pair_kernel<bf16_t>, grid, dim3(256), 0, s, q);
+                else hipLaunchKernelGGL(gemm_pair_kernel<f16_t>, grid, dim3(256), 0, s, q);
+            } else if (a->N == 64) {
+                if (bf) hipLaunchKernelGGL((gemm_pair_ln_kernel<bf16_t, 64>), grid, dim3(256), 0, s, q);
+                else hipLaunchKernelGGL((gemm_pair_ln_kernel<f16_t, 64>), grid, dim3(256), 0, s, q);
+            } else {
+                if (bf) hipLaunchKernelGGL((gemm_pair_ln_kernel<bf16_t, 128>), grid, dim3(256), 0, s, q);
+                else hipLaunchKernelGGL((gemm_pair_ln_kernel<f16_t, 128>), grid, dim3(256), 0, s, q);
+            }
             return tc_launch_status();
         }
     }
-    const int rc = tc_gemm(a, stream);
+    const int rc = ln ? tc_gemm_ln(a, ln, stream) : tc_gemm(a, stream);
     return rc != TC_OK ? rc : tc_gemm(b, stream);
 }
 
-extern "C" int tc_gemm_multi(const TcGemm* g, int n, void* stream) {
+extern "C" int tc_gemm_pair(const TcGemm* a, const TcGemm* b, void* stream) { return gemm_pair_impl(a, nullptr, b, stream); }
+
+extern "C" int tc_gemm_ln_supported(int C, int dtype) { return (C == 64 || C == 128) && (dtype == TC_BF16 || dtype == TC_F16); }
+
+extern "C" int tc_gemm_ln(const TcGemm* g, const TcGemmLn* ln, void* stream) {
+    if (!gemm_args_ok(g) || !gemm_ln_args_ok(g, ln)) return TC_ERR_ARG;
+    hipStream_t s = (hipStream_t)stream;
+    if (g->dtype == TC_BF16) return gemm_typed<bf16_t>(g, s, ln);
+    return gemm_typed<f16_t>(g, s, ln);
+}
+
+extern "C" int tc_gemm_pair_ln(const TcGemm* a, const TcGemmLn* ln, const TcGemm* b, void* stream) {
+    if (!ln) return TC_ERR_ARG;
+    return gemm_pair_impl(a, ln, b, stream);
+}
+
+static int gemm_multi_impl(const TcGemm* g, const TcGemmLn* ln, int n, void* stream);
+extern "C" int tc_gemm_multi(const TcGemm* g, int n, void* stream) { return gemm_multi_impl(g, nullptr, n, stream); }
+extern "C" int tc_gemm_multi_ln(const TcGemm* g, const TcGemmLn* ln, int n, void* stream) {
+    if (!ln) return TC_ERR_ARG;
+    return gemm_multi_impl(g, ln, n, stream);
+}
+
+static int gemm_multi_impl(const TcGemm* g, const TcGemmLn* ln, int n, void* stream) {
     if (!g || n < 1) return TC_ERR_ARG;
-    for (int i = 0; i < n; ++i) if (!gemm_args_ok(g + i) || g[i].bn_part) return TC_ERR_ARG;
+    for (int i = 0; i < n; ++i) if (!gemm_args_ok(g + i) || g[i].bn_part || (ln && ln[i].x && !gemm_ln_args_ok(g + i, ln + i))) return TC_ERR_ARG;
     hipStream_t s = (hipStream_t)stream;
     bool ok = n <= GEMM_MULTI_MAX;
     GemmMultiDev q;
@@ -1178,8 +1358,10 @@
         if (h16 && !t.transA && t.transB && !t.c_f32) kind = t.ffn_mode == TC_FFN_LN_A ? 3 : (t.ffn_mode ? -1 : 0);
         else if (h16 && !t.transA && !t.transB && !t.c_f32) kind = t.ffn_mode == TC_FFN_EP ? 4 : (t.ffn_mode ? -1 : 1);
         else if (h16 && t.transA && !t.transB && t.c_f32) kind = t.ffn_mode == TC_FFN_LN_B ? 5 : (t.ffn_mode ? -1 : 2);
+        const TcGemmLn* li = (ln && ln[i].x) ? ln + i : nullptr;
+        if (li) kind = (kind == 1 && t.N == 64) ? 6 : -1;
         bool big;
-        if (kind < 0 || !gemm_plan<bf16_t>(&t, plan[i], grids[i], big, true)) { ok = false; break; }
+        if (kind < 0 || !gemm_plan<bf16_t>(&t, plan[i], grids[i], big, true, li)) { ok = false; break; }
         kinds[i] = kind; order[i] = i;
     }
     long long blk = 0;
@@ -1201,7 +1383,7 @@
         return tc_launch_status();
     }
     for (int i = 0; i < n; ++i) {
-        const int rc = tc_gemm(g + i, stream);
+        const int rc = (ln && ln[i].x) ? tc_gemm_ln(g + i, ln + i, stream) : tc_gemm(g + i, stream);
         if (rc != TC_OK) return rc;
     }
     return TC_OK;
diff --git a/transception_amd/csrc/norm.hip b/transception_amd/csrc/norm.hip
--- a/transception_amd/csrc/norm.hip
+++ b/transception_amd/csrc/norm.hip
@@ -13,13 +13,6 @@
     return deferred ? LN_BWD_MAX_BLOCKS : 1024;
 }
 
-struct LnMap { int p, H, W; };
-__device__ __forceinline__ long long ln_row_off(int row, const LnMap& m, int ld, int C) {
-    if (m.p == 0) return (long long)row * ld;
-    const int Wp = m.W * m.p, Hp = m.H * m.p;
-    const int ow = row % Wp, t = row / Wp, oh = t % Hp, b = t / Hp;
-    return ((long long)(b * m.H + oh / m.p) * m.W + ow / m.p) * ld + ((oh % m.p) * m.p + ow % m.p) * C;
-}
 
 template <int GS> __device__ __forceinline__ float group_sum(float v) { return tc_group_sum<GS>(v); }
 
diff --git a/transception_amd/csrc/tc_common.h b/transception_amd/csrc/tc_common.h
--- a/transception_amd/csrc/tc_common.h
+++ b/transception_amd/csrc/tc_common.h
@@ -107,6 +107,14 @@
     if (G >= 32) v = fmaxf(v, __shfl_xor(v, 16, 64));
     if (G >= 64) v = fmaxf(v, __shfl_xor(v, 32, 64));
     return v;
+}
+
+struct LnMap { int p, H, W; };
+__device__ __forceinline__ long long ln_row_off(int row, const LnMap& m, int ld, int C) {
+    if (m.p == 0) return (long long)row * ld;
+    const int Wp = m.W * m.p, Hp = m.H * m.p;
+    const int ow = row % Wp, t = row / Wp, oh = t % Hp, b = t / Hp;
+    return ((long long)(b * m.H + oh / m.p) * m.W + ow / m.p) * ld + ((oh % m.p) * m.p + ow % m.p) * C;
 }
 
 __device__ __forceinline__ int tc_mul24(int a, int b) { return a * b; }
diff --git a/transception_amd/engine.py b/transception_amd/engine.py
--- a/transception_amd/engine.py
+++ b/transception_amd/engine.py
@@ -7,7 +7,7 @@
 import torch
 
 from ._lib import (ATTN_DKV_SPLITS, EW_COPY, EW_DEINTERLEAVE, EW_PATCHIFY, TcEffAtt, TcEwSeg, TcFfnBwd, TcFfnFused, ACT_COORD, ACT_GELU, ACT_HSWISH, ACT_NONE, ACT_SCALE, ACT_SIGMOID, FFN_EP, FFN_LN_A, FFN_LN_B, TC_BF16, TC_F16, TC_F32, TcDwSeg, TcFfnSeg,
-                   TcGemm, lib)
+                   TcGemm, TcGemmLn, lib)
 
 _DT = {torch.float32: TC_F32, torch.bfloat16: TC_BF16, torch.float16: TC_F16}
 
@@ -40,11 +40,12 @@
     return fl, by
 
 
-def _timed_gemm(kind: str, descs, fn):
+def _timed_gemm(kind: str, descs, fn, extra_bytes: float = 0.0):
     if PROFILE is None:
         fn()
         return
-    _timed("gemm:" + kind, _gemm_work(descs), fn)
+    fl, by = _gemm_work(descs)
+    _timed("gemm:" + kind, (fl, by + extra_bytes), fn)
 
 
 class P:
@@ -57,7 +58,8 @@
 
 
 class Var:
-    __slots__ = ("data", "root", "path", "kids", "grad_t", "whole_written", "written", "requires_grad", "region", "reshaped", "covered", "bn_part")
+    __slots__ = ("data", "root", "path", "kids", "grad_t", "whole_written", "written", "requires_grad", "region", "reshaped", "covered", "bn_part",
+                 "ln_site")
 
     def __init__(self, data: torch.Tensor, root: "Var" = None, path=None, requires_grad: bool = True, region=None,
                  reshaped: bool = False):
@@ -73,6 +75,7 @@
         self.region = region if region is not None else (0, data.shape[0], 0, data.shape[1])
         self.covered = False
         self.reshaped = reshaped
+        self.ln_site: Optional[dict] = None
 
     rows = property(lambda s: s.data.shape[0])
     cols = property(lambda s: s.data.shape[1])
@@ -388,6 +391,37 @@
         tiles = ((m_out + 63) // 64) * ((n_out + 63) // 64)
         cap = _SPLITK_CAP if k_red < 262144 else 1024
         return max(1, min(max(_SPLITK_BLOCKS, cap) // max(tiles, 1), k_red // _SPLITK_KMIN, cap))
+
+    def _ln_fusable(self, x: Var, M: int, nb: int, batch, side_by_side: bool) -> Optional[dict]:
+        st = x.ln_site
+        if st is None or st["linears"] != 1 or self.dt == TC_F32 or batch is not None or side_by_side or st["act"] != ACT_NONE:
+            return None
+        t = st["x"]
+        if (not t.requires_grad or not x.is_whole or x.root.grad_t is not None or st["Gn"] != nb or st["rows"] != M
+                or not bool(self.L.tc_gemm_ln_supported(st["C"], self.dt))):
+            return None
+        tg = t.root.grad_t
+        if t.ld % 8 or t.data.data_ptr() % 16 or st["g"].data.data_ptr() % 16 or (nb > 1 and st["g"].gs % 8):
+            return None
+        if tg is not None and (t.apply_path(tg).data_ptr() % 16 or t.apply_path(tg).stride(0) % 8):
+            return None
+        if nb > 1 and not t.data.is_contiguous():
+            return None
+        return st
+
+    def _ln_desc(self, st: dict, gt: torch.Tensor, tacc: int, M: int, nb: int):
+        t, g, b, Cc = st["x"], st["g"], st["b"], st["C"]
+        es = t.data.element_size()
+        part, nf, nblk = None, 0, (M + 63) // 64
+        if g.grad is not None:
+            nf = nb * nblk * 2 * Cc
+            part = self.f32(nf)
+            self._ln_pending.append((part, g.grad, b.grad, g.gs, nblk, Cc, nb))
+            if len(self._ln_pending) == 64:
+                self._flush_param_folds()
+        lnd = TcGemmLn(_ptr(t.data), _ptr(gt) if tacc else None, _ptr(g.data), _ptr(st["mean"]), _ptr(st["rstd"]), _ptr(part), nf,
+                       g.gs if nb > 1 else 0, t.ld, gt.stride(0), 0, 0, 0, 0)
+        return lnd, (1.0 + tacc) * nb * M * Cc * es
 
     def linear(self, x: Var, W: P, b: Optional[P] = None, out: Optional[Var] = None, residual: Optional[Var] = None,
                act: int = ACT_NONE, wcols: Optional[Tuple[int, int]] = None, accumulate: bool = False,
@@ -415,6 +449,8 @@
             sw = 0
         if post_scale is not None:
             assert act == ACT_NONE and not accumulate
+        if x.ln_site is not None:
+            x.ln_site["linears"] += 1
         bn_part = None
         if (bn_shift is not None and self.training and self.dtype != torch.float32 and nb == 1 and not accumulate
                 and act == ACT_NONE and post_scale is None and N % 8 == 0 and out.ld % 8 == 0 and out.data.data_ptr() % 16 == 0):
@@ -440,7 +476,29 @@
             want_db = b is not None and b.grad is not None
             paired = (x.requires_grad and W.grad is not None and self.dtype != torch.float32
                       and self._small_tiles(M, K, nb) and self._small_tiles(N, K, nb))
-            if paired:
+            ln = self._ln_fusable(x, M, nb, batch, side_by_side) if x.requires_grad else None
+            if ln is not None:
+                st = x.ln_site
+                t = st["x"]
+                gt, tacc = self.wgrad(t)
+                lnd, lnb = self._ln_desc(st, gt, tacc, M, nb)
+                ga = self._gemm_desc(_ptr(dz), dz.stride(0), _ptr(Wt), Wt.stride(0), _ptr(gt), gt.stride(0), M, K, N, 0, 0,
+                                     nb1=nb, sA=(so, 0), sB=(sw, 0), sC=(M * gt.stride(0) if nb > 1 else 0, 0), use_ws=False)
+                self.n_launch += 1
+                if W.grad is not None and self._small_tiles(N, K, nb):
+                    gW = W.grad if wcols is None else W.grad[:, wcols[0]:wcols[1]]
+                    gb = self._gemm_desc(_ptr(dz), dz.stride(0), _ptr(x.data), x.ld, _ptr(gW), gW.stride(0), N, K, M, 1, 0, acc=1,
+                                         splitk=self._splitk(N, K, M), c_f32=1, nb1=nb, sA=(so, 0), sB=(sx, 0), sC=(sw, 0),
+                                         rowsum=_ptr(b.grad) if want_db else None, srow=sw, use_ws=False)
+                    if gb.splitk > 128:
+                        ws = _workspace(self.dev)
+                        gb.ws, gb.ws_bytes = ws.data_ptr(), ws.numel()
+                    _timed_gemm("pair", [ga, gb], lambda: self.L.tc_gemm_pair_ln(C.byref(ga), C.byref(lnd), C.byref(gb), self.stream), lnb)
+                    paired = True
+                else:
+                    _timed_gemm("single", [ga], lambda: self.L.tc_gemm_ln(C.byref(ga), C.byref(lnd), self.stream), lnb)
+                    paired = False
+            elif paired:
                 gx, acc = self.wgrad(x, (nb - 1) * sx // x.root.cols if (nb > 1 and not grouped) else 0)
                 gW = W.grad if wcols is None else W.grad[:, wcols[0]:wcols[1]]
                 ga = self._gemm_desc(_ptr(dz), dz.stride(0), _ptr(Wt), Wt.stride(0), _ptr(gx), gx.stride(0), M, K, N, 0, 0, acc=acc,
@@ -453,7 +511,7 @@
                     gb.ws, gb.ws_bytes, ga.ws, ga.ws_bytes = ga.ws, ga.ws_bytes, None, 0
                 self.n_launch += 1
                 _timed_gemm("pair", [ga, gb], lambda: self.L.tc_gemm_pair(C.byref(ga), C.byref(gb), self.stream))
-            elif x.requires_grad:
+            elif x.requires_grad and ln is None:
                 gx, acc = self.wgrad(x, (nb - 1) * sx // x.root.cols if (nb > 1 and not grouped) else 0)
                 self._gemm(_ptr(dz), dz.stride(0), _ptr(Wt), Wt.stride(0), _ptr(gx), gx.stride(0), M, K, N, 0, 0, acc=acc,
                            nb1=nb, sA=(so, 0), sB=(sw, 0), sC=(sx, 0))
@@ -894,6 +952,8 @@
                 _ptr(x.data), x.ld, _ptr(g.data), _ptr(b.data), _ptr(out.data), out.ld, _ptr(mean), _ptr(rstd), rows, Cc, eps, act, Gn, g.gs,
                 self.dt, self.stream))
 
+        out.ln_site = {"x": x, "g": g, "b": b, "mean": mean, "rstd": rstd, "rows": rows, "C": Cc, "Gn": Gn, "act": act, "linears": 0}
+
         def bwd():
             dy = self.grad_of(out)
             if dy is None or not x.requires_grad:
```

New measurement: 1494 images/sec, median of 6. 2.2% higher.
